# hugofloresgarcia/ddsp_pytorch

Hardware: NVIDIA B200
Metric: DDSP synth audio samples/sec (fwd+bwd) (higher is better)
Workload: dtype f32

## Files before the change

ddsp_pytorch_b200/csrc/noise.cu:

```cuda
#include "common.cuh"

namespace {

constexpr int kNoiseThreads = 128;

__device__ __forceinline__ void ir_design_row(const float *m, const float *ct, float *h, int NB,
                                              int tid, int nthr) {
    const int half = NB - 1, F = 2 * half;
    const float invF = 1.f / (float)F;
    for (int n = tid; 2 * n <= half; n += nthr) {
        float ev = 0.f, od = 0.f;
        int idx = 0;
        for (int k = 0; k < NB; ++k) {
            const float ck = (k == 0 || k == half) ? 1.f : 2.f;
            const float t = ck * m[k] * ct[idx];
            if (k & 1) od += t; else ev += t;
            idx += n;
            if (idx >= F) idx -= F;
        }
        h[n] = (ev + od) * invF;
        h[half - n] = (ev - od) * invF;
    }
}

__device__ __forceinline__ void ir_design_row_bwd(const float *dh, const float *ct, float *dm, int NB,
                                                  int tid, int nthr) {
    const int half = NB - 1, F = 2 * half;
    const float invF = 1.f / (float)F;
    for (int k = tid; k < NB; k += nthr) {
        float acc = 0.f;
        int idx = 0;
        for (int n = 0; n <= half; ++n) {
            acc = fmaf(dh[n], ct[idx], acc);
            idx += k;
            if (idx >= F) idx -= F;
        }
        dm[k] = acc * invF * ((k == 0 || k == half) ? 1.f : 2.f);
    }
}

__device__ __forceinline__ float hann_periodic(int i, int F) {
    return 0.5f - 0.5f * cospif(2.f * (float)i / (float)F);
}

template <bool BWD>
__global__ void __launch_bounds__(kNoiseThreads)
amp_to_ir_kernel(const float *__restrict__ in, float *__restrict__ out, int64_t rows, int NB,
                 int target) {
    extern __shared__ __align__(16) float smem[];
    const int half = NB - 1, F = 2 * half;
    float *ct = smem;
    float *m = ct + F;
    float *h = m + NB;
    const int tid = threadIdx.x;
    for (int i = tid; i < F; i += kNoiseThreads) ct[i] = cospif(2.f * (float)i / (float)F);
    const int lim = min(F, target);
    for (int64_t row = blockIdx.x; row < rows; row += gridDim.x) {
        __syncthreads();
        if (!BWD) {
            for (int k = tid; k < NB; k += kNoiseThreads) m[k] = in[row * NB + k];
            __syncthreads();
            ir_design_row(m, ct, h, NB, tid, kNoiseThreads);
            __syncthreads();
            for (int i = tid; i < target; i += kNoiseThreads) {
                int j = i + half;
                j = j % target;
                float v = 0.f;
                if (j < lim) {
                    int n = j - half;
                    if (n < 0) n += F;
                    n = min(n, F - n);
                    v = h[n] * hann_periodic(j, F);
                }
                out[row * target + i] = v;
            }
        } else {
            for (int n = tid; n <= half; n += kNoiseThreads) h[n] = 0.f;
            __syncthreads();
            for (int i = tid; i < target; i += kNoiseThreads) {
                int j = (i + half) % target;
                if (j < lim) {
                    int n = j - half;
                    if (n < 0) n += F;
                    n = min(n, F - n);
                    atomicAdd(&h[n], in[row * target + i] * hann_periodic(j, F));
                }
            }
            __syncthreads();
            ir_design_row_bwd(h, ct, m, NB, tid, kNoiseThreads);
            __syncthreads();
            for (int k = tid; k < NB; k += kNoiseThreads) out[row * NB + k] = m[k];
        }
    }
}

struct NoiseLayout {
    int NBp, HP, F, half, bs, stride;
    __host__ __device__ NoiseLayout(int NB, int bs_) {
        half = NB - 1; F = 2 * half; bs = bs_;
        NBp = (NB + 3) & ~3; HP = (half + 1 + 3) & ~3;
        stride = NBp + HP + F + (half + bs) + bs;
        stride = (stride + 3) & ~3;
    }
    __host__ __device__ int m() const { return 0; }
    __host__ __device__ int h() const { return NBp; }
    __host__ __device__ int taps() const { return NBp + HP; }
    __host__ __device__ int xs() const { return NBp + HP + F; }
    __host__ __device__ int ys() const { return NBp + HP + F + half + bs; }
};

__global__ void __launch_bounds__(kNoiseThreads)
filtered_noise_fwd_kernel(const float *__restrict__ mags, const float *__restrict__ noise,
                          const float *__restrict__ add, float *__restrict__ out, int64_t rows, int NB,
                          int bs, int RPC, int apply_scale, float bias) {
    extern __shared__ __align__(16) float smem[];
    const NoiseLayout L(NB, bs);
    const int half = L.half, F = L.F;
    float *ct = smem;
    float *rowbase = smem + ((F + 3) & ~3);
    const int tid = threadIdx.x;
    for (int i = tid; i < F; i += kNoiseThreads) ct[i] = cospif(2.f * (float)i / (float)F);

    const int QT = bs >> 2;
    for (int64_t r0 = (int64_t)blockIdx.x * RPC; r0 < rows; r0 += (int64_t)gridDim.x * RPC) {
        const int nr = (int)min((int64_t)RPC, rows - r0);
        __syncthreads();
        for (int i = tid; i < nr * NB; i += kNoiseThreads) {
            const int r = i / NB, k = i - r * NB;
            const float m = __ldg(mags + (r0 + r) * NB + k);
            rowbase[r * L.stride + L.m() + k] = apply_scale ? ddsp_scale_fn(m + bias) : m;
        }
        for (int i = tid; i < nr * (half + bs); i += kNoiseThreads) {
            const int r = i / (half + bs), j = i - r * (half + bs);
            rowbase[r * L.stride + L.xs() + j] = j < half ? 0.f : __ldg(noise + (r0 + r) * bs + (j - half));
        }
        __syncthreads();
        {
            const int per = kNoiseThreads / nr;
            const int r = tid / per, t = tid - r * per;
            if (r < nr) {
                float *rb = rowbase + r * L.stride;
                ir_design_row(rb + L.m(), ct, rb + L.h(), NB, t, per);
            }
        }
        __syncthreads();
        for (int i = tid; i < nr * F; i += kNoiseThreads) {
            const int r = i / F, d = i - r * F;
            float *rb = rowbase + r * L.stride;
            const float *h = rb + L.h();
            rb[L.taps() + d] = d < half ? h[d] * hann_periodic(d + half, F)
                                        : h[F - d] * hann_periodic(d - half, F);
        }
        __syncthreads();
        for (int w = tid; w < nr * QT; w += kNoiseThreads) {
            const int r = w / QT, i = (w - r * QT) * 4;
            const float *rb = rowbase + r * L.stride;
            const float4 *c4 = reinterpret_cast<const float4 *>(rb + L.taps());
            const float *xs = rb + L.xs() + half + i;
            float y0 = 0.f, y1 = 0.f, y2 = 0.f, y3 = 0.f;
            float4 hi = *reinterpret_cast<const float4 *>(xs);
            for (int d = 0; d < half; d += 4) {
                const float4 lo = *reinterpret_cast<const float4 *>(xs - d - 4);
                const float4 c = c4[d >> 2];
                y0 = fmaf(c.x, hi.x, y0); y1 = fmaf(c.x, hi.y, y1); y2 = fmaf(c.x, hi.z, y2); y3 = fmaf(c.x, hi.w, y3);
                y0 = fmaf(c.y, lo.w, y0); y1 = fmaf(c.y, hi.x, y1); y2 = fmaf(c.y, hi.y, y2); y3 = fmaf(c.y, hi.z, y3);
                y0 = fmaf(c.z, lo.z, y0); y1 = fmaf(c.z, lo.w, y1); y2 = fmaf(c.z, hi.x, y2); y3 = fmaf(c.z, hi.y, y3);
                y0 = fmaf(c.w, lo.y, y0); y1 = fmaf(c.w, lo.z, y1); y2 = fmaf(c.w, lo.w, y2); y3 = fmaf(c.w, hi.x, y3);
                hi = lo;
            }
            *reinterpret_cast<float4 *>(const_cast<float *>(rb) + L.ys() + i) = make_float4(y0, y1, y2, y3);
        }
        __syncthreads();
        for (int w = tid; w < nr * half; w += kNoiseThreads) {
            const int r = w / half, t = w - r * half;
            float *rb = rowbase + r * L.stride;
            const float *far = rb + L.taps() + half;
            const float *x = rb + L.xs() + half;
            float acc = 0.f;
            for (int e = 1; e <= t; ++e) acc = fmaf(far[e], x[t - e], acc);
            rb[L.ys() + bs - half + t] += acc;
        }
        __syncthreads();
        for (int i = tid; i < nr * bs; i += kNoiseThreads) {
            const int r = i / bs, j = i - r * bs;
            float y = rowbase[r * L.stride + L.ys() + j];
            if (add) y += __ldg(add + (r0 + r) * bs + j);
            out[(r0 + r) * bs + j] = y;
        }
    }
}

__global__ void __launch_bounds__(kNoiseThreads)
filtered_noise_bwd_kernel(const float *__restrict__ g_out, const float *__restrict__ noise,
                          const float *__restrict__ mags_raw, float *__restrict__ d_mags, int64_t rows,
                          int NB, int bs, int RPC, int apply_scale, float bias) {
    extern __shared__ __align__(16) float smem[];
    const NoiseLayout L(NB, bs);
    const int half = L.half, F = L.F;
    float *ct = smem;
    float *rowbase = smem + ((F + 3) & ~3);
    const int tid = threadIdx.x;
    for (int i = tid; i < F; i += kNoiseThreads) ct[i] = cospif(2.f * (float)i / (float)F);

    for (int64_t r0 = (int64_t)blockIdx.x * RPC; r0 < rows; r0 += (int64_t)gridDim.x * RPC) {
        const int nr = (int)min((int64_t)RPC, rows - r0);
        __syncthreads();
        for (int i = tid; i < nr * (half + bs); i += kNoiseThreads) {
            const int r = i / (half + bs), j = i - r * (half + bs);
            rowbase[r * L.stride + L.xs() + j] = j < half ? 0.f : __ldg(noise + (r0 + r) * bs + (j - half));
        }
        for (int i = tid; i < nr * bs; i += kNoiseThreads) {
            const int r = i / bs, j = i - r * bs;
            rowbase[r * L.stride + L.ys() + j] = __ldg(g_out + (r0 + r) * bs + j);
        }
        __syncthreads();
        for (int w = tid; w < nr * F; w += kNoiseThreads) {
            const int r = w / F, d = w - r * F;
            float *rb = rowbase + r * L.stride;
            const float *g = rb + L.ys();
            const float *x = rb + L.xs() + half;
            float a0 = 0.f, a1 = 0.f;
            if (d < half) {
                int i = 0;
                for (; i + 1 < bs; i += 2) {
                    a0 = fmaf(g[i], x[i - d], a0);
                    a1 = fmaf(g[i + 1], x[i + 1 - d], a1);
                }
                if (i < bs) a0 = fmaf(g[i], x[i - d], a0);
            } else {
                const int e = d - half;
                if (e >= 1)
                    for (int t = e; t < half; ++t) a0 = fmaf(g[bs - half + t], x[t - e], a0);
            }
            rb[L.taps() + d] = a0 + a1;
        }
        __syncthreads();
        for (int w = tid; w < nr * (half + 1); w += kNoiseThreads) {
            const int r = w / (half + 1), n = w - r * (half + 1);
            float *rb = rowbase + r * L.stride;
            const float *dt = rb + L.taps();
            float v = 0.f;
            if (n < half) v = dt[n] * hann_periodic(n + half, F);
            const int e = half - n;
            if (e >= 1 && e < half) v = fmaf(dt[half + e], hann_periodic(e, F), v);
            rb[L.h() + n] = v;
        }
        __syncthreads();
        {
            const int per = kNoiseThreads / nr;
            const int r = tid / per, t = tid - r * per;
            if (r < nr) {
                float *rb = rowbase + r * L.stride;
                ir_design_row_bwd(rb + L.h(), ct, rb + L.m(), NB, t, per);
            }
        }
        __syncthreads();
        for (int i = tid; i < nr * NB; i += kNoiseThreads) {
            const int r = i / NB, k = i - r * NB;
            float d = rowbase[r * L.stride + L.m() + k];
            if (apply_scale) d *= ddsp_scale_grad(__ldg(mags_raw + (r0 + r) * NB + k) + bias);
            d_mags[(r0 + r) * NB + k] = d;
        }
    }
}

constexpr int kN2Threads = 256;

__global__ void noise_design_kernel(float *__restrict__ tab, int NB) {
    const int half = NB - 1, F = 2 * half, NBq = (NB + 3) & ~3;
    const int total = NB * F;
    for (int i = blockIdx.x * blockDim.x + threadIdx.x; i < total; i += gridDim.x * blockDim.x) {
        const int k = i / F, j = i - k * F;
        const int n = j < half ? j : half - (j - half);
        const int wi = j < half ? j + half : j - half;
        const double ck = (k == 0 || k == half) ? 1.0 : 2.0;
        const double c = ck * cospi(2.0 * (double)((k * n) % F) / F) / F;
        const double w = 0.5 - 0.5 * cospi(2.0 * (double)wi / F);
        const float v = (float)(c * w);
        tab[i] = v;
        tab[(size_t)total + (size_t)j * NBq + k] = v;
    }
    for (int i = blockIdx.x * blockDim.x + threadIdx.x; i < F * (NBq - NB); i += gridDim.x * blockDim.x) {
        const int j = i / (NBq - NB), k = NB + i % (NBq - NB);
        tab[(size_t)total + (size_t)j * NBq + k] = 0.f;
    }
}

__device__ __forceinline__ float4 fir4(const float4 *__restrict__ t4, const float *x, int ntaps) {
    float y0 = 0.f, y1 = 0.f, y2 = 0.f, y3 = 0.f;
    float4 hi = *reinterpret_cast<const float4 *>(x);
    for (int d = 0; d < ntaps; d += 4) {
        const float4 lo = *reinterpret_cast<const float4 *>(x - d - 4);
        const float4 c = t4[d >> 2];
        y0 = fmaf(c.x, hi.x, y0); y1 = fmaf(c.x, hi.y, y1); y2 = fmaf(c.x, hi.z, y2); y3 = fmaf(c.x, hi.w, y3);
        y0 = fmaf(c.y, lo.w, y0); y1 = fmaf(c.y, hi.x, y1); y2 = fmaf(c.y, hi.y, y2); y3 = fmaf(c.y, hi.z, y3);
        y0 = fmaf(c.z, lo.z, y0); y1 = fmaf(c.z, lo.w, y1); y2 = fmaf(c.z, hi.x, y2); y3 = fmaf(c.z, hi.y, y3);
        y0 = fmaf(c.w, lo.y, y0); y1 = fmaf(c.w, lo.z, y1); y2 = fmaf(c.w, lo.w, y2); y3 = fmaf(c.w, hi.x, y3);
        hi = lo;
    }
    return make_float4(y0, y1, y2, y3);
}

__device__ __forceinline__ float4 corr4(const float *g, const float *x, int d, int len) {
    float a0 = 0.f, a1 = 0.f, a2 = 0.f, a3 = 0.f;
    float4 lo = *reinterpret_cast<const float4 *>(x - d - 4);
    for (int i = 0; i < len; i += 4) {
        const float4 hi = *reinterpret_cast<const float4 *>(x + i - d);
        const float4 gv = *reinterpret_cast<const float4 *>(g + i);
        a0 = fmaf(gv.x, hi.x, a0); a0 = fmaf(gv.y, hi.y, a0); a0 = fmaf(gv.z, hi.z, a0); a0 = fmaf(gv.w, hi.w, a0);
        a1 = fmaf(gv.x, lo.w, a1); a1 = fmaf(gv.y, hi.x, a1); a1 = fmaf(gv.z, hi.y, a1); a1 = fmaf(gv.w, hi.z, a1);
        a2 = fmaf(gv.x, lo.z, a2); a2 = fmaf(gv.y, lo.w, a2); a2 = fmaf(gv.z, hi.x, a2); a2 = fmaf(gv.w, hi.y, a2);
        a3 = fmaf(gv.x, lo.y, a3); a3 = fmaf(gv.y, lo.z, a3); a3 = fmaf(gv.z, lo.w, a3); a3 = fmaf(gv.w, hi.x, a3);
        lo = hi;
    }
    return make_float4(a0, a1, a2, a3);
}

struct Noise2Layout {
    int half, F, NBq, bs, xs_len, stride;
    __host__ __device__ Noise2Layout(int NB, int bs_) {
        half = NB - 1; F = 2 * half; NBq = (NB + 3) & ~3; bs = bs_;
        xs_len = half + bs;
        stride = NBq + F + xs_len + bs + half;
    }
    __host__ __device__ int m() const { return 0; }
    __host__ __device__ int taps() const { return NBq; }
    __host__ __device__ int xs() const { return NBq + F; }
    __host__ __device__ int ys() const { return NBq + F + xs_len; }
    __host__ __device__ int yf() const { return NBq + F + xs_len + bs; }
};

__global__ void __launch_bounds__(kN2Threads)
filtered_noise2_fwd_kernel(const float *__restrict__ mags, const float *__restrict__ noise,
                           const float *__restrict__ add, const float *__restrict__ design,
                           float *__restrict__ out, int64_t rows, int NB, int bs, int RPC, int apply_scale,
                           float bias) {
    extern __shared__ __align__(16) float smem[];
    const Noise2Layout L(NB, bs);
    const int half = L.half, F = L.F;
    float *D = smem;
    float *rowbase = D + NB * F;
    const int tid = threadIdx.x, warp = tid >> 5, lane = tid & 31;
    constexpr int NW = kN2Threads / 32;
    for (int i = tid; i < NB * F / 4; i += kN2Threads)
        reinterpret_cast<float4 *>(D)[i] = __ldg(reinterpret_cast<const float4 *>(design) + i);

    const int QM = bs >> 2, QF = half >> 2;
    for (int64_t r0 = (int64_t)blockIdx.x * RPC; r0 < rows; r0 += (int64_t)gridDim.x * RPC) {
        const int nr = (int)min((int64_t)RPC, rows - r0);
        __syncthreads();
        for (int r = warp; r < nr; r += NW) {
            float *rb = rowbase + r * L.stride;
            const float *mg = mags + (r0 + r) * NB;
            for (int k = lane; k < NB; k += 32) {
                const float m = __ldg(mg + k);
                rb[L.m() + k] = apply_scale ? ddsp_scale_fn(m + bias) : m;
            }
            for (int j = lane; j < half; j += 32) rb[L.xs() + j] = 0.f;
            const float4 *nz = reinterpret_cast<const float4 *>(noise + (r0 + r) * bs);
            float4 *xs4 = reinterpret_cast<float4 *>(rb + L.xs() + half);
            for (int j = lane; j < QM; j += 32) xs4[j] = __ldg(nz + j);
        }
        __syncthreads();
        for (int it = tid; it < ((nr + 1) >> 1) * (F / 4); it += kN2Threads) {
            const int rp = it / (F / 4), c = it - rp * (F / 4);
            const int ra = 2 * rp, rb_ = min(2 * rp + 1, nr - 1);
            const float *ma = rowbase + ra * L.stride + L.m();
            const float *mb = rowbase + rb_ * L.stride + L.m();
            const float4 *d4 = reinterpret_cast<const float4 *>(D) + c;
            float4 a = make_float4(0.f, 0.f, 0.f, 0.f), e = a;
#define DDSP_N2_MAC(X, Y, U)                                                                                  \
    a.x = fmaf(X, U.x, a.x); a.y = fmaf(X, U.y, a.y); a.z = fmaf(X, U.z, a.z); a.w = fmaf(X, U.w, a.w);      \
    e.x = fmaf(Y, U.x, e.x); e.y = fmaf(Y, U.y, e.y); e.z = fmaf(Y, U.z, e.z); e.w = fmaf(Y, U.w, e.w);
            for (int k = 0; k < NB - 1; k += 4) {
                const float4 xa = *reinterpret_cast<const float4 *>(ma + k);
                const float4 xb = *reinterpret_cast<const float4 *>(mb + k);
                const float4 u0 = d4[k * (F / 4)], u1 = d4[(k + 1) * (F / 4)];
                const float4 u2 = d4[(k + 2) * (F / 4)], u3 = d4[(k + 3) * (F / 4)];
                DDSP_N2_MAC(xa.x, xb.x, u0)
                DDSP_N2_MAC(xa.y, xb.y, u1)
                DDSP_N2_MAC(xa.z, xb.z, u2)
                DDSP_N2_MAC(xa.w, xb.w, u3)
            }
            {
                const float4 u = d4[(NB - 1) * (F / 4)];
                const float x = ma[NB - 1], y = mb[NB - 1];
                DDSP_N2_MAC(x, y, u)
            }
#undef DDSP_N2_MAC
            reinterpret_cast<float4 *>(rowbase + ra * L.stride + L.taps())[c] = a;
            if (rb_ != ra) reinterpret_cast<float4 *>(rowbase + rb_ * L.stride + L.taps())[c] = e;
        }
        __syncthreads();
        const int nmain = nr * QM;
        for (int it = tid; it < nmain + nr * QF; it += kN2Threads) {
            if (it < nmain) {
                const int r = it / QM, q = it - r * QM;
                float *rb = rowbase + r * L.stride;
                const float4 y = fir4(reinterpret_cast<const float4 *>(rb + L.taps()), rb + L.xs() + half + 4 * q, half);
                *reinterpret_cast<float4 *>(rb + L.ys() + 4 * q) = y;
            } else {
                const int i2 = it - nmain;
                const int r = i2 / QF, qq = i2 - r * QF;
                float *rb = rowbase + r * L.stride;
                const float4 y = fir4(reinterpret_cast<const float4 *>(rb + L.taps()) + QF,
                                      rb + L.xs() + half + 4 * qq, half);
                *reinterpret_cast<float4 *>(rb + L.yf() + 4 * qq) = y;
            }
        }
        __syncthreads();
        for (int r = warp; r < nr; r += NW) {
            const float *rb = rowbase + r * L.stride;
            const float4 *ys4 = reinterpret_cast<const float4 *>(rb + L.ys());
            const float4 *yf4 = reinterpret_cast<const float4 *>(rb + L.yf());
            const float4 *ad4 = add ? reinterpret_cast<const float4 *>(add + (r0 + r) * bs) : nullptr;
            float4 *o4 = reinterpret_cast<float4 *>(out + (r0 + r) * bs);
            for (int j = lane; j < QM; j += 32) {
                float4 y = ys4[j];
                if (j >= QM - QF) {
                    const float4 f = yf4[j - (QM - QF)];
                    y.x += f.x; y.y += f.y; y.z += f.z; y.w += f.w;
                }
                if (ad4) {
                    const float4 f = __ldg(ad4 + j);
                    y.x += f.x; y.y += f.y; y.z += f.z; y.w += f.w;
                }
                o4[j] = y;
            }
        }
    }
}

__global__ void __launch_bounds__(kN2Threads)
filtered_noise2_bwd_kernel(const float *__restrict__ g_out, const float *__restrict__ noise,
                           const float *__restrict__ mags_raw, const float *__restrict__ design,
                           float *__restrict__ d_mags, int64_t rows, int NB, int bs, int RPC,
                           int apply_scale, float bias) {
    extern __shared__ __align__(16) float smem[];
    const Noise2Layout L(NB, bs);
    const int half = L.half, F = L.F, NBq = L.NBq;
    float *Dt = smem;
    float *rowbase = Dt + F * NBq;
    const int tid = threadIdx.x, warp = tid >> 5, lane = tid & 31;
    constexpr int NW = kN2Threads / 32;
    const float *dt_src = design + (size_t)NB * F;
    for (int i = tid; i < F * NBq / 4; i += kN2Threads)
        reinterpret_cast<float4 *>(Dt)[i] = __ldg(reinterpret_cast<const float4 *>(dt_src) + i);
    const int QM = bs >> 2;

    for (int64_t r0 = (int64_t)blockIdx.x * RPC; r0 < rows; r0 += (int64_t)gridDim.x * RPC) {
        const int nr = (int)min((int64_t)RPC, rows - r0);
        __syncthreads();
        for (int r = warp; r < nr; r += NW) {
            float *rb = rowbase + r * L.stride;
            for (int j = lane; j < half; j += 32) rb[L.xs() + j] = 0.f;
            const float4 *nz = reinterpret_cast<const float4 *>(noise + (r0 + r) * bs);
            const float4 *gz = reinterpret_cast<const float4 *>(g_out + (r0 + r) * bs);
            float4 *xs4 = reinterpret_cast<float4 *>(rb + L.xs() + half);
            float4 *g4 = reinterpret_cast<float4 *>(rb + L.ys());
            for (int j = lane; j < QM; j += 32) {
                xs4[j] = __ldg(nz + j);
                g4[j] = __ldg(gz + j);
            }
        }
        __syncthreads();
        const int ncausal = nr * (half / 4);
        for (int it = tid; it < 2 * ncausal; it += kN2Threads) {
            const bool far = it >= ncausal;
            const int i2 = far ? it - ncausal : it;
            const int r = i2 / (half / 4), tg = i2 - r * (half / 4);
            float *rb = rowbase + r * L.stride;
            const float *x = rb + L.xs() + half;
            const float4 a = far ? corr4(rb + L.ys() + bs - half, x, 4 * tg, half) : corr4(rb + L.ys(), x, 4 * tg, bs);
            *reinterpret_cast<float4 *>(rb + L.taps() + (far ? half : 0) + 4 * tg) = a;
        }
        __syncthreads();
        for (int it = tid; it < ((nr + 1) >> 1) * (NBq / 4); it += kN2Threads) {
            const int rp = it / (NBq / 4), kg = it - rp * (NBq / 4);
            const int ra = 2 * rp, rb_ = min(2 * rp + 1, nr - 1);
            const float *ta = rowbase + ra * L.stride + L.taps();
            const float *tb = rowbase + rb_ * L.stride + L.taps();
            const float4 *d4 = reinterpret_cast<const float4 *>(Dt) + kg;
            float4 a = make_float4(0.f, 0.f, 0.f, 0.f), e = a;
#define DDSP_N2_MAC(X, Y, U)                                                                                  \
    a.x = fmaf(X, U.x, a.x); a.y = fmaf(X, U.y, a.y); a.z = fmaf(X, U.z, a.z); a.w = fmaf(X, U.w, a.w);      \
    e.x = fmaf(Y, U.x, e.x); e.y = fmaf(Y, U.y, e.y); e.z = fmaf(Y, U.z, e.z); e.w = fmaf(Y, U.w, e.w);
            for (int j = 0; j < F; j += 4) {
                const float4 xa = *reinterpret_cast<const float4 *>(ta + j);
                const float4 xb = *reinterpret_cast<const float4 *>(tb + j);
                const float4 u0 = d4[j * (NBq / 4)], u1 = d4[(j + 1) * (NBq / 4)];
                const float4 u2 = d4[(j + 2) * (NBq / 4)], u3 = d4[(j + 3) * (NBq / 4)];
                DDSP_N2_MAC(xa.x, xb.x, u0)
                DDSP_N2_MAC(xa.y, xb.y, u1)
                DDSP_N2_MAC(xa.z, xb.z, u2)
                DDSP_N2_MAC(xa.w, xb.w, u3)
            }
#undef DDSP_N2_MAC
#pragma unroll
            for (int h2 = 0; h2 < 2; ++h2) {
                if (h2 == 1 && rb_ == ra) break;
                const int r = h2 ? rb_ : ra;
                const float4 acc = h2 ? e : a;
                const float av[4] = {acc.x, acc.y, acc.z, acc.w};
#pragma unroll
                for (int q = 0; q < 4; ++q) {
                    const int k = 4 * kg + q;
                    if (k < NB) {
                        float d = av[q];
                        if (apply_scale) d *= ddsp_scale_grad(__ldg(mags_raw + (r0 + r) * NB + k) + bias);
                        d_mags[(r0 + r) * NB + k] = d;
                    }
                }
            }
        }
    }
}

inline int noise_rows_per_cta(int bs) {
    int rpc = (kNoiseThreads * 4) / bs;
    if (rpc < 1) rpc = 1;
    if (rpc > 8) rpc = 8;
    return rpc;
}

}

extern "C" int ddsp_b200_amp_to_ir_fwd(const float *amp, float *ir, int64_t rows, int NB, int target,
                                       void *stream) {
    DDSP_REQUIRE(amp && ir && rows >= 0 && NB >= 2 && target >= 1);
    if (rows == 0) return DDSP_B200_OK;
    const size_t smem = (size_t)(2 * (NB - 1) + NB + NB) * sizeof(float);
    if (smem > 48 * 1024) return DDSP_B200_EUNSUPPORTED;
    const int grid = (int)(rows < DDSP_SM_COUNT * 16 ? rows : DDSP_SM_COUNT * 16);
    amp_to_ir_kernel<false><<<grid, kNoiseThreads, smem, (cudaStream_t)stream>>>(amp, ir, rows, NB,
                                                                                 target);
    return ddsp_launch_status();
}

extern "C" int ddsp_b200_amp_to_ir_bwd(const float *d_ir, float *d_amp, int64_t rows, int NB,
                                       int target, void *stream) {
    DDSP_REQUIRE(d_ir && d_amp && rows >= 0 && NB >= 2 && target >= 1);
    if (rows == 0) return DDSP_B200_OK;
    const size_t smem = (size_t)(2 * (NB - 1) + NB + NB) * sizeof(float);
    if (smem > 48 * 1024) return DDSP_B200_EUNSUPPORTED;
    const int grid = (int)(rows < DDSP_SM_COUNT * 16 ? rows : DDSP_SM_COUNT * 16);
    amp_to_ir_kernel<true><<<grid, kNoiseThreads, smem, (cudaStream_t)stream>>>(d_ir, d_amp, rows,
                                                                                NB, target);
    return ddsp_launch_status();
}

static int noise_launch_cfg(int64_t rows, int NB, int bs, int *rpc, size_t *smem, int *grid) {
    if (NB < 3 || (NB - 1) % 4 != 0) return DDSP_B200_EUNSUPPORTED;
    if (bs % 4 != 0 || bs < 2 * (NB - 1)) return DDSP_B200_EUNSUPPORTED;
    *rpc = noise_rows_per_cta(bs);
    const NoiseLayout L(NB, bs);
    *smem = ((size_t)((L.F + 3) & ~3) + (size_t)*rpc * L.stride) * sizeof(float);
    if (*smem > 200 * 1024) return DDSP_B200_EUNSUPPORTED;
    const int64_t ctas = ddsp_ceil_div(rows, *rpc);
    *grid = (int)(ctas < DDSP_SM_COUNT * 8 ? ctas : DDSP_SM_COUNT * 8);
    return DDSP_B200_OK;
}

static bool noise2_cfg(int64_t rows, int NB, int bs, bool bwd, int *rpc, size_t *smem, int *grid) {
    if (NB < 5 || (NB - 1) % 4 != 0 || bs % 4 != 0 || bs < 2 * (NB - 1)) return false;
    const Noise2Layout L(NB, bs);
    const size_t fixed = (bwd ? (size_t)L.F * L.NBq : (size_t)NB * L.F) * sizeof(float);
    int r = 16;
    while (r > 1 && fixed + (size_t)r * L.stride * sizeof(float) > 75 * 1024) r >>= 1;
    *smem = fixed + (size_t)r * L.stride * sizeof(float);
    if (*smem > 200 * 1024) return false;
    *rpc = r;
    const int64_t ctas = ddsp_ceil_div(rows, r);
    *grid = (int)(ctas < DDSP_SM_COUNT * 3 ? ctas : DDSP_SM_COUNT * 3);
    return true;
}

extern "C" int64_t ddsp_b200_noise_design_size(int NB) {
    if (NB < 2) return 0;
    const int F = 2 * (NB - 1), NBq = (NB + 3) & ~3;
    return (int64_t)NB * F + (int64_t)F * NBq;
}

extern "C" int ddsp_b200_noise_design_table(float *table, int NB, void *stream) {
    DDSP_REQUIRE(table && NB >= 2);
    noise_design_kernel<<<64, 256, 0, (cudaStream_t)stream>>>(table, NB);
    return ddsp_launch_status();
}

extern "C" int ddsp_b200_filtered_noise_fwd(const float *mags, const float *noise, const float *add,
                                            const float *design, float *out, int64_t rows, int NB,
                                            int block_size, int apply_scale, float bias, void *stream) {
    DDSP_REQUIRE(mags && noise && out && rows >= 0);
    if (rows == 0) return DDSP_B200_OK;
    int rpc, grid;
    size_t smem;
    if (design && noise2_cfg(rows, NB, block_size, false, &rpc, &smem, &grid)) {
        if (smem > 48 * 1024)
            cudaFuncSetAttribute(filtered_noise2_fwd_kernel, cudaFuncAttributeMaxDynamicSharedMemorySize,
                                 (int)smem);
        filtered_noise2_fwd_kernel<<<grid, kN2Threads, smem, (cudaStream_t)stream>>>(
            mags, noise, add, design, out, rows, NB, block_size, rpc, apply_scale, bias);
        return ddsp_launch_status();
    }
    int s = noise_launch_cfg(rows, NB, block_size, &rpc, &smem, &grid);
    if (s) return s;
    if (smem > 48 * 1024)
        cudaFuncSetAttribute(filtered_noise_fwd_kernel, cudaFuncAttributeMaxDynamicSharedMemorySize,
                             (int)smem);
    filtered_noise_fwd_kernel<<<grid, kNoiseThreads, smem, (cudaStream_t)stream>>>(
        mags, noise, add, out, rows, NB, block_size, rpc, apply_scale, bias);
    return ddsp_launch_status();
}

extern "C" int ddsp_b200_filtered_noise_bwd(const float *g_out, const float *noise,
                                            const float *mags_raw, const float *design, float *d_mags,
                                            int64_t rows, int NB, int block_size, int apply_scale,
                                            float bias, void *stream) {
    DDSP_REQUIRE(g_out && noise && d_mags && rows >= 0 && (!apply_scale || mags_raw));
    if (rows == 0) return DDSP_B200_OK;
    int rpc, grid;
    size_t smem;
    if (design && noise2_cfg(rows, NB, block_size, true, &rpc, &smem, &grid)) {
        if (smem > 48 * 1024)
            cudaFuncSetAttribute(filtered_noise2_bwd_kernel, cudaFuncAttributeMaxDynamicSharedMemorySize,
                                 (int)smem);
        filtered_noise2_bwd_kernel<<<grid, kN2Threads, smem, (cudaStream_t)stream>>>(
            g_out, noise, mags_raw, design, d_mags, rows, NB, block_size, rpc, apply_scale, bias);
        return ddsp_launch_status();
    }
    int s = noise_launch_cfg(rows, NB, block_size, &rpc, &smem, &grid);
    if (s) return s;
    if (smem > 48 * 1024)
        cudaFuncSetAttribute(filtered_noise_bwd_kernel, cudaFuncAttributeMaxDynamicSharedMemorySize,
                             (int)smem);
    filtered_noise_bwd_kernel<<<grid, kNoiseThreads, smem, (cudaStream_t)stream>>>(
        g_out, noise, mags_raw, d_mags, rows, NB, block_size, rpc, apply_scale, bias);
    return ddsp_launch_status();
}
```

ddsp_pytorch_b200/csrc/torch_ops.cpp:

```cpp
#include <ATen/ATen.h>
#include <ATen/cuda/CUDAContext.h>
#include <ATen/cuda/CUDAEvent.h>
#include <c10/cuda/CUDAGuard.h>
#include <c10/cuda/CUDAStream.h>
#include <torch/library.h>

#include <map>
#include <mutex>
#include <tuple>
#include <vector>

#include "ddsp_b200.h"

namespace {

using at::Tensor;

void check(int status, const char *what) {
    TORCH_CHECK(status == DDSP_B200_OK, "ddsp_b200::", what, " failed: ", ddsp_b200_strerror(status),
                " (status ", status, ")");
}

Tensor prep(const Tensor &t, const char *name) {
    TORCH_CHECK(t.is_cuda(), "ddsp_b200: ", name, " must be a CUDA tensor (no CPU fallback exists)");
    TORCH_CHECK(t.scalar_type() == at::kFloat, "ddsp_b200: ", name, " must be float32, got ",
                t.scalar_type());
    return t.contiguous();
}

void *cur_stream() { return (void *)at::cuda::getCurrentCUDAStream().stream(); }
const float *fp(const Tensor &t) { return t.data_ptr<float>(); }
float *fpm(Tensor &t) { return t.data_ptr<float>(); }

void finish_table_build(const char *what) {
    cudaStreamCaptureStatus cap = cudaStreamCaptureStatusNone;
    cudaStream_t st = at::cuda::getCurrentCUDAStream().stream();
    TORCH_CHECK(cudaStreamIsCapturing(st, &cap) == cudaSuccess && cap == cudaStreamCaptureStatusNone,
                "ddsp_b200: constant table '", what, "' would be built inside a CUDA graph capture; run the op "
                "once eagerly (warm-up) before capturing");
    TORCH_CHECK(cudaStreamSynchronize(st) == cudaSuccess, "ddsp_b200: building table '", what, "' failed");
}

Tensor twiddle_table(const at::Device &dev, int64_t n) {
    static std::mutex mu;
    static std::map<std::pair<int, int64_t>, Tensor> cache;
    std::lock_guard<std::mutex> lock(mu);
    auto key = std::make_pair((int)dev.index(), n);
    auto it = cache.find(key);
    if (it != cache.end()) return it->second;
    Tensor t = at::empty({n, 2}, at::TensorOptions().device(dev).dtype(at::kFloat));
    check(ddsp_b200_twiddle_table(fpm(t), (int)n, cur_stream()), "twiddle_table");
    finish_table_build("twiddle_table");
    cache[key] = t;
    return t;
}

Tensor stage_twiddle_table(const at::Device &dev, int64_t n_fft) {
    static std::mutex mu;
    static std::map<std::pair<int, int64_t>, Tensor> cache;
    std::lock_guard<std::mutex> lock(mu);
    auto key = std::make_pair((int)dev.index(), n_fft);
    auto it = cache.find(key);
    if (it != cache.end()) return it->second;
    const int64_t n = ddsp_b200_fft_stage_twiddles_size((int)n_fft);
    Tensor t;
    if (n > 0) {
        t = at::empty({n, 2}, at::TensorOptions().device(dev).dtype(at::kFloat));
        check(ddsp_b200_fft_stage_twiddles(fpm(t), (int)n_fft, cur_stream()), "stft_stage_twiddles");
        finish_table_build("fft_stage_twiddles");
    }
    cache[key] = t;
    return t;
}

Tensor noise_design_table(const at::Device &dev, int64_t NB) {
    static std::mutex mu;
    static std::map<std::pair<int, int64_t>, Tensor> cache;
    std::lock_guard<std::mutex> lock(mu);
    auto key = std::make_pair((int)dev.index(), NB);
    auto it = cache.find(key);
    if (it != cache.end()) return it->second;
    Tensor t = at::empty({ddsp_b200_noise_design_size((int)NB)}, at::TensorOptions().device(dev).dtype(at::kFloat));
    check(ddsp_b200_noise_design_table(fpm(t), (int)NB, cur_stream()), "noise_design_table");
    finish_table_build("noise_design_table");
    cache[key] = t;
    return t;
}

Tensor scale_function_fwd(const Tensor &x_) {
    Tensor x = prep(x_, "x");
    c10::cuda::CUDAGuard guard(x.device());
    Tensor y = at::empty_like(x);
    check(ddsp_b200_scale_function_fwd(fp(x), fpm(y), x.numel(), cur_stream()), "scale_function_fwd");
    return y;
}

Tensor scale_function_bwd(const Tensor &x_, const Tensor &dy_) {
    Tensor x = prep(x_, "x"), dy = prep(dy_, "dy");
    TORCH_CHECK(x.numel() == dy.numel(), "scale_function_bwd: size mismatch");
    c10::cuda::CUDAGuard guard(x.device());
    Tensor dx = at::empty_like(x);
    check(ddsp_b200_scale_function_bwd(fp(x), fp(dy), fpm(dx), x.numel(), cur_stream()),
          "scale_function_bwd");
    return dx;
}

Tensor remove_above_nyquist(const Tensor &amp_, const Tensor &f0_, double sample_rate) {
    Tensor amp = prep(amp_, "amplitudes"), f0 = prep(f0_, "f0");
    TORCH_CHECK(amp.dim() >= 1 && f0.numel() * amp.size(-1) == amp.numel(),
                "remove_above_nyquist: f0 must have one value per row of amplitudes");
    c10::cuda::CUDAGuard guard(amp.device());
    Tensor out = at::empty_like(amp);
    check(ddsp_b200_remove_above_nyquist(fp(amp), fp(f0), fpm(out), f0.numel(), (int)amp.size(-1),
                                         (float)sample_rate, cur_stream()),
          "remove_above_nyquist");
    return out;
}

Tensor opt_prep(const c10::optional<Tensor> &t, const char *name) {
    return (t.has_value() && t->defined()) ? prep(*t, name) : Tensor();
}
const float *opt_fp(const Tensor &t) { return t.defined() ? t.data_ptr<float>() : nullptr; }

std::tuple<Tensor, Tensor, Tensor> harmonic_controls_fwd(const Tensor &amp_raw_, const Tensor &dist_raw_,
                                                         const Tensor &f0_, double sample_rate,
                                                         bool with_weights) {
    Tensor a = prep(amp_raw_, "amplitudes"), d = prep(dist_raw_, "harmonic_distribution"),
           f = prep(f0_, "f0");
    const int64_t H = d.size(-1), rows = d.numel() / H;
    TORCH_CHECK(a.numel() == rows && f.numel() == rows, "harmonic_controls: shape mismatch");
    c10::cuda::CUDAGuard guard(d.device());
    Tensor amps = at::empty_like(a), dist = at::empty_like(d);
    Tensor weights = with_weights ? at::empty_like(d) : at::empty({0}, d.options());
    check(ddsp_b200_harmonic_controls_fwd(fp(a), fp(d), fp(f), fpm(amps), fpm(dist),
                                          with_weights ? fpm(weights) : nullptr, rows, (int)H,
                                          (float)sample_rate, cur_stream()),
          "harmonic_controls_fwd");
    return {amps, dist, weights};
}

std::tuple<Tensor, Tensor> harmonic_controls_bwd(const Tensor &amp_raw_, const Tensor &dist_raw_,
                                                 const Tensor &f0_, const c10::optional<Tensor> &d_amps_,
                                                 const c10::optional<Tensor> &d_dist_,
                                                 const c10::optional<Tensor> &d_weights_,
                                                 double sample_rate) {
    Tensor a = prep(amp_raw_, "amplitudes"), d = prep(dist_raw_, "harmonic_distribution"),
           f = prep(f0_, "f0");
    Tensor ga = opt_prep(d_amps_, "d_amps"), gd = opt_prep(d_dist_, "d_dist"),
           gw = opt_prep(d_weights_, "d_weights");
    const int64_t H = d.size(-1), rows = d.numel() / H;
    TORCH_CHECK(a.numel() == rows && f.numel() == rows && (!ga.defined() || ga.numel() == rows) &&
                    (!gd.defined() || gd.numel() == d.numel()) && (!gw.defined() || gw.numel() == d.numel()),
                "harmonic_controls_bwd: shape mismatch");
    c10::cuda::CUDAGuard guard(d.device());
    Tensor da = at::empty_like(a), dd = at::empty_like(d);
    check(ddsp_b200_harmonic_controls_bwd(fp(a), fp(d), fp(f), opt_fp(ga), opt_fp(gd), opt_fp(gw), fpm(da),
                                          fpm(dd), rows, (int)H, (float)sample_rate, cur_stream()),
          "harmonic_controls_bwd");
    return {da, dd};
}

std::tuple<Tensor, Tensor, Tensor, Tensor> harmonic_fwd(const Tensor &f0_, const Tensor &weights_,
                                                        int64_t block_size, double sample_rate,
                                                        const c10::optional<Tensor> &phase0_) {
    Tensor f0 = prep(f0_, "f0"), w = prep(weights_, "weights");
    TORCH_CHECK(w.dim() == 3, "harmonic_fwd: weights must be (B,T,H)");
    const int64_t B = w.size(0), T = w.size(1), H = w.size(2);
    TORCH_CHECK(f0.numel() == B * T, "harmonic_fwd: f0 must be (B,T,1)");
    c10::cuda::CUDAGuard guard(w.device());
    auto opt64 = w.options().dtype(at::kLong);
    Tensor phi = at::empty({B, T}, opt64), delta = at::empty({B, T}, opt64);
    Tensor phase_end = at::empty({B}, w.options().dtype(at::kDouble));
    Tensor audio = at::empty({B, T * block_size, 1}, w.options());
    if (B == 0 || T == 0) return {audio, phase_end.zero_(), phi, delta};
    const double *p0 = nullptr;
    Tensor phase0;
    if (phase0_.has_value() && phase0_->defined()) {
        phase0 = phase0_->contiguous();
        TORCH_CHECK(phase0.is_cuda() && phase0.scalar_type() == at::kDouble && phase0.numel() == B,
                    "harmonic_fwd: phase0 must be a CUDA float64 tensor of B turns");
        p0 = phase0.data_ptr<double>();
    }
    check(ddsp_b200_phase_scan(fp(f0), p0, (uint64_t *)phi.data_ptr<int64_t>(),
                               (uint64_t *)delta.data_ptr<int64_t>(), phase_end.data_ptr<double>(),
                               (int)B, (int)T, (int)block_size, sample_rate, cur_stream()),
          "phase_scan");
    check(ddsp_b200_harmonic_frames_fwd(fp(w), (const uint64_t *)phi.data_ptr<int64_t>(),
                                        (const uint64_t *)delta.data_ptr<int64_t>(), fpm(audio), (int)B,
                                        (int)T, (int)H, (int)block_size, cur_stream()),
          "harmonic_frames_fwd");
    return {audio, phase_end, phi, delta};
}

std::tuple<Tensor, Tensor> harmonic_bwd(const Tensor &g_, const Tensor &weights_, const Tensor &phi,
                                        const Tensor &delta, int64_t block_size, double sample_rate,
                                        bool need_f0) {
    Tensor g = prep(g_, "grad_audio"), w = prep(weights_, "weights");
    const int64_t B = w.size(0), T = w.size(1), H = w.size(2);
    TORCH_CHECK(g.numel() == B * T * block_size, "harmonic_bwd: grad shape mismatch");
    TORCH_CHECK(phi.is_cuda() && phi.scalar_type() == at::kLong && phi.is_contiguous() &&
                    delta.is_cuda() && delta.scalar_type() == at::kLong && delta.is_contiguous() &&
                    phi.numel() == B * T && delta.numel() == B * T,
                "harmonic_bwd: bad phase workspace");
    c10::cuda::CUDAGuard guard(w.device());
    Tensor dw = at::empty_like(w);
    if (B == 0 || T == 0) return {dw, at::empty({B, T, 1}, w.options())};
    const uint64_t *ph = (const uint64_t *)phi.data_ptr<int64_t>();
    const uint64_t *dl = (const uint64_t *)delta.data_ptr<int64_t>();
    check(ddsp_b200_harmonic_frames_bwd_weights(fp(g), ph, dl, fpm(dw), (int)B, (int)T, (int)H,
                                                (int)block_size, cur_stream()),
          "harmonic_frames_bwd_weights");
    Tensor df0;
    if (need_f0) {
        df0 = at::empty({B, T, 1}, w.options());
        Tensor scratch = at::empty({B, T, 2}, w.options());
        check(ddsp_b200_harmonic_frames_bwd_f0(fp(g), fp(w), ph, dl, fpm(scratch), fpm(df0), (int)B, (int)T,
                                               (int)H, (int)block_size, sample_rate, cur_stream()),
              "harmonic_frames_bwd_f0");
    } else {
        df0 = at::empty({0}, w.options());
    }
    return {dw, df0};
}

int64_t harmonic_raw_supported(int64_t H, int64_t block_size) {
    return ddsp_b200_harmonic_frames_raw_supported((int)H, (int)block_size);
}

struct RawViews {
    Tensor first, dist;
    const float *amp, *dst;
    int64_t amp_stride, dist_stride, B, T, H;
    bool joint;
};

RawViews raw_views(const Tensor &first_, const c10::optional<Tensor> &dist_raw_) {
    RawViews v;
    v.first = prep(first_, "amplitudes / projection");
    v.joint = !(dist_raw_.has_value() && dist_raw_->defined());
    TORCH_CHECK(v.first.dim() == 3, "harmonic_raw: expected (B,T,.) tensors");
    v.B = v.first.size(0);
    v.T = v.first.size(1);
    if (v.joint) {
        v.H = v.first.size(2) - 1;
        TORCH_CHECK(v.H >= 1, "harmonic_raw: the projection must be (B,T,H+1)");
        v.amp = fp(v.first);
        v.dst = v.amp + 1;
        v.amp_stride = v.dist_stride = v.H + 1;
    } else {
        v.dist = prep(*dist_raw_, "harmonic_distribution");
        TORCH_CHECK(v.dist.dim() == 3 && v.dist.size(0) == v.B && v.dist.size(1) == v.T && v.first.size(2) == 1,
                    "harmonic_raw: amplitudes (B,T,1) and harmonic_distribution (B,T,H) expected");
        v.H = v.dist.size(2);
        v.amp = fp(v.first);
        v.dst = fp(v.dist);
        v.amp_stride = 1;
        v.dist_stride = v.H;
    }
    return v;
}

std::tuple<Tensor, Tensor, Tensor, Tensor, Tensor, Tensor> harmonic_raw_fwd(
    const Tensor &first_, const c10::optional<Tensor> &dist_raw_, const Tensor &f0_, int64_t block_size,
    double sample_rate, const c10::optional<Tensor> &phase0_) {
    RawViews v = raw_views(first_, dist_raw_);
    Tensor f0 = prep(f0_, "f0");
    const int64_t B = v.B, T = v.T, H = v.H;
    TORCH_CHECK(f0.numel() == B * T, "harmonic_raw_fwd: f0 must be (B,T,1)");
    c10::cuda::CUDAGuard guard(f0.device());
    auto opt = f0.options();
    Tensor phi = at::empty({B, T}, opt.dtype(at::kLong)), delta = at::empty({B, T}, opt.dtype(at::kLong));
    Tensor phase_end = at::empty({B}, opt.dtype(at::kDouble));
    Tensor audio = at::empty({B, T * block_size, 1}, opt);
    Tensor amps = at::empty({B, T, 1}, opt), weights = at::empty({B, T, H}, opt);
    if (B == 0 || T == 0) return {audio, phase_end.zero_(), phi, delta, amps, weights};
    const double *p0 = nullptr;
    Tensor phase0;
    if (phase0_.has_value() && phase0_->defined()) {
        phase0 = phase0_->contiguous();
        TORCH_CHECK(phase0.is_cuda() && phase0.scalar_type() == at::kDouble && phase0.numel() == B,
                    "harmonic_raw_fwd: phase0 must be a CUDA float64 tensor of B turns");
        p0 = phase0.data_ptr<double>();
    }
    check(ddsp_b200_harmonic_frames_raw_scan_fwd(v.amp, v.amp_stride, v.dst, v.dist_stride, fp(f0), p0,
                                                 (uint64_t *)phi.data_ptr<int64_t>(),
                                                 (uint64_t *)delta.data_ptr<int64_t>(), phase_end.data_ptr<double>(),
                                                 fpm(amps), fpm(weights), fpm(audio), (int)B, (int)T, (int)H,
                                                 (int)block_size, sample_rate, cur_stream()),
          "harmonic_frames_raw_scan_fwd");
    return {audio, phase_end, phi, delta, amps, weights};
}

std::tuple<Tensor, Tensor> harmonic_raw_bwd(const Tensor &g_, const Tensor &first_,
                                            const c10::optional<Tensor> &dist_raw_, const Tensor &f0_,
                                            const Tensor &phi, const Tensor &delta, int64_t block_size,
                                            double sample_rate) {
    RawViews v = raw_views(first_, dist_raw_);
    Tensor g = prep(g_, "grad_audio"), f0 = prep(f0_, "f0");
    const int64_t B = v.B, T = v.T, H = v.H;
    TORCH_CHECK(g.numel() == B * T * block_size && f0.numel() == B * T, "harmonic_raw_bwd: shape mismatch");
    TORCH_CHECK(phi.is_cuda() && phi.scalar_type() == at::kLong && phi.is_contiguous() &&
                    delta.is_cuda() && delta.scalar_type() == at::kLong && delta.is_contiguous() &&
                    phi.numel() == B * T && delta.numel() == B * T,
                "harmonic_raw_bwd: bad phase workspace");
    c10::cuda::CUDAGuard guard(g.device());
    Tensor d0, d1;
    float *da, *dd;
    int64_t das, dds;
    if (v.joint) {
        d0 = at::empty({B, T, H + 1}, g.options());
        d1 = at::empty({0}, g.options());
        da = fpm(d0);
        dd = da + 1;
        das = dds = H + 1;
    } else {
        d0 = at::empty({B, T, 1}, g.options());
        d1 = at::empty({B, T, H}, g.options());
        da = fpm(d0);
        dd = fpm(d1);
        das = 1;
        dds = H;
    }
    if (B == 0 || T == 0) return {d0, d1};
    check(ddsp_b200_harmonic_frames_raw_bwd(fp(g), v.amp, v.amp_stride, v.dst, v.dist_stride, fp(f0),
                                            (const uint64_t *)phi.data_ptr<int64_t>(),
                                            (const uint64_t *)delta.data_ptr<int64_t>(), da, das, dd, dds, (int)B,
                                            (int)T, (int)H, (int)block_size, (float)sample_rate, cur_stream()),
          "harmonic_frames_raw_bwd");
    return {d0, d1};
}

std::tuple<Tensor, Tensor> harmonic_ar_fwd(const Tensor &f0_, const Tensor &amps_, double sample_rate) {
    Tensor f0 = prep(f0_, "f0"), a = prep(amps_, "amplitudes");
    TORCH_CHECK(a.dim() == 3, "harmonic_synth: amplitudes must be (B,N,H)");
    const int64_t B = a.size(0), N = a.size(1), H = a.size(2);
    TORCH_CHECK(f0.numel() == B * N, "harmonic_synth: f0 must be (B,N,1)");
    c10::cuda::CUDAGuard guard(a.device());
    Tensor phase = at::empty({B, N}, a.options().dtype(at::kLong));
    Tensor audio = at::empty({B, N, 1}, a.options());
    check(ddsp_b200_phase_scan_audio_rate(fp(f0), (uint64_t *)phase.data_ptr<int64_t>(), (int)B, N,
                                          sample_rate, cur_stream()),
          "phase_scan_audio_rate");
    check(ddsp_b200_harmonic_audio_rate_fwd(fp(a), (const uint64_t *)phase.data_ptr<int64_t>(), fpm(audio),
                                            (int)B, N, (int)H, cur_stream()),
          "harmonic_audio_rate_fwd");
    return {audio, phase};
}

std::tuple<Tensor, Tensor> harmonic_ar_bwd(const Tensor &g_, const Tensor &amps_, const Tensor &phase,
                                           double sample_rate, bool need_f0) {
    Tensor g = prep(g_, "grad_audio"), a = prep(amps_, "amplitudes");
    const int64_t B = a.size(0), N = a.size(1), H = a.size(2);
    TORCH_CHECK(g.numel() == B * N && phase.numel() == B * N && phase.scalar_type() == at::kLong &&
                    phase.is_cuda() && phase.is_contiguous(),
                "harmonic_synth backward: shape mismatch");
    c10::cuda::CUDAGuard guard(a.device());
    Tensor da = at::empty_like(a);
    Tensor df0 = need_f0 ? at::empty({B, N, 1}, a.options()) : at::empty({0}, a.options());
    Tensor dphi = need_f0 ? at::empty({B, N}, a.options()) : Tensor();
    check(ddsp_b200_harmonic_audio_rate_bwd(fp(g), fp(a), (const uint64_t *)phase.data_ptr<int64_t>(),
                                            fpm(da), need_f0 ? fpm(dphi) : nullptr,
                                            need_f0 ? fpm(df0) : nullptr, (int)B, N, (int)H, sample_rate,
                                            cur_stream()),
          "harmonic_audio_rate_bwd");
    return {da, df0};
}

Tensor amp_to_ir_fwd(const Tensor &amp_, int64_t target) {
    Tensor amp = prep(amp_, "amp");
    const int64_t NB = amp.size(-1), rows = amp.numel() / NB;
    c10::cuda::CUDAGuard guard(amp.device());
    auto shape = amp.sizes().vec();
    shape.back() = target;
    Tensor ir = at::empty(shape, amp.options());
    check(ddsp_b200_amp_to_ir_fwd(fp(amp), fpm(ir), rows, (int)NB, (int)target, cur_stream()),
          "amp_to_ir_fwd");
    return ir;
}

Tensor amp_to_ir_bwd(const Tensor &d_ir_, int64_t NB) {
    Tensor d_ir = prep(d_ir_, "d_ir");
    const int64_t target = d_ir.size(-1), rows = d_ir.numel() / target;
    c10::cuda::CUDAGuard guard(d_ir.device());
    auto shape = d_ir.sizes().vec();
    shape.back() = NB;
    Tensor d_amp = at::empty(shape, d_ir.options());
    check(ddsp_b200_amp_to_ir_bwd(fp(d_ir), fpm(d_amp), rows, (int)NB, (int)target, cur_stream()),
          "amp_to_ir_bwd");
    return d_amp;
}

Tensor noise_fwd(const Tensor &mags_, const Tensor &noise_, const c10::optional<Tensor> &add_, bool apply_scale,
                 double bias) {
    Tensor mags = prep(mags_, "magnitudes"), noise = prep(noise_, "noise"), add = opt_prep(add_, "add");
    TORCH_CHECK(mags.dim() == 3 && noise.dim() == 3 && mags.size(0) == noise.size(0) &&
                    mags.size(1) == noise.size(1),
                "filtered noise: magnitudes (B,T,NB) and noise (B,T,block) expected");
    const int64_t B = mags.size(0), T = mags.size(1), NB = mags.size(2), bs = noise.size(2);
    TORCH_CHECK(!add.defined() || add.numel() == B * T * bs, "filtered noise: `add` must be (B,T*block,1)");
    c10::cuda::CUDAGuard guard(mags.device());
    Tensor out = at::empty({B, T * bs, 1}, mags.options());
    if (B * T == 0) return out;
    Tensor design = noise_design_table(mags.device(), NB);
    check(ddsp_b200_filtered_noise_fwd(fp(mags), fp(noise), opt_fp(add), fp(design), fpm(out), B * T, (int)NB,
                                       (int)bs, apply_scale, (float)bias, cur_stream()),
          "filtered_noise_fwd");
    return out;
}

Tensor noise_bwd(const Tensor &g_, const Tensor &noise_, const c10::optional<Tensor> &mags_raw_, int64_t NB,
                 bool apply_scale, double bias) {
    Tensor g = prep(g_, "grad_out"), noise = prep(noise_, "noise"), raw = opt_prep(mags_raw_, "mags_raw");
    const int64_t B = noise.size(0), T = noise.size(1), bs = noise.size(2);
    TORCH_CHECK(g.numel() == B * T * bs, "filtered noise backward: shape mismatch");
    TORCH_CHECK(!apply_scale || (raw.defined() && raw.numel() == B * T * NB),
                "filtered noise backward: raw magnitudes needed when the scale function is fused");
    c10::cuda::CUDAGuard guard(noise.device());
    Tensor d_mags = at::empty({B, T, NB}, noise.options());
    if (B * T == 0) return d_mags;
    Tensor design = noise_design_table(noise.device(), NB);
    check(ddsp_b200_filtered_noise_bwd(fp(g), fp(noise), opt_fp(raw), fp(design), fpm(d_mags), B * T, (int)NB,
                                       (int)bs, apply_scale, (float)bias, cur_stream()),
          "filtered_noise_bwd");
    return d_mags;
}

struct ConvPlan {
    int n1, n2;
    int64_t n;
    Tensor tw, st1, st2;
};

ConvPlan conv_plan(const at::Device &dev, int64_t min_len) {
    ConvPlan p;
    check(ddsp_b200_conv_plan(min_len, &p.n1, &p.n2), "conv_plan");
    p.n = (int64_t)p.n1 * p.n2;
    p.tw = twiddle_table(dev, p.n);
    p.st1 = stage_twiddle_table(dev, p.n1);
    p.st2 = stage_twiddle_table(dev, p.n2);
    return p;
}

Tensor fftconv_spectrum(const Tensor &kernel_, int64_t n_signal) {
    Tensor ker = prep(kernel_, "kernel");
    TORCH_CHECK(ker.dim() == 2 && n_signal > 0, "fftconv_spectrum: 2-D (rows, length) kernel expected");
    const int64_t Rk = ker.size(0), Lk = ker.size(1);
    c10::cuda::CUDAGuard guard(ker.device());
    const int64_t Lc = std::min(Lk, n_signal);
    Tensor kc = Lc == Lk ? ker : ker.narrow(1, 0, Lc).contiguous();
    ConvPlan p = conv_plan(ker.device(), n_signal + Lc - 1);
    void *st = cur_stream();
    Tensor hspec = at::empty({Rk, p.n, 2}, ker.options());
    check(ddsp_b200_fft4_cols_fwd(fp(kc), Rk, Lc, 0, fpm(hspec), fp(p.tw), opt_fp(p.st1), p.n1, p.n2, st), "fft4_cols_fwd(h)");
    check(ddsp_b200_fft4_rows_spectrum(fpm(hspec), Rk, fp(p.tw), fp(p.st2), p.n1, p.n2, st), "fft4_rows_spectrum");
    return hspec;
}

std::tuple<Tensor, Tensor, Tensor> fftconv_fwd(const Tensor &signal_, const Tensor &kernel_, bool keep,
                                               const c10::optional<Tensor> &hspec_,
                                               const c10::optional<Tensor> &signal2_) {
    Tensor sig = prep(signal_, "signal"), ker = prep(kernel_, "kernel");
    Tensor sig2 = opt_prep(signal2_, "signal2");
    TORCH_CHECK(!sig2.defined() || sig2.sizes() == sig.sizes(), "fftconv: signal2 must have the signal's shape");
    TORCH_CHECK(sig.dim() == 2 && ker.dim() == 2, "fftconv: 2-D (rows, length) tensors expected");
    const int64_t R = sig.size(0), n = sig.size(1), Rk = ker.size(0), Lk = ker.size(1);
    TORCH_CHECK(Rk == 1 || Rk == R, "fftconv: kernel rows must be 1 or match the signal rows");
    c10::cuda::CUDAGuard guard(sig.device());
    Tensor out = at::empty_like(sig);
    Tensor none = at::empty({0}, sig.options());
    if (R == 0 || n == 0) return {out, none, none};
    const int64_t Lc = std::min(Lk, n);
    ConvPlan p = conv_plan(sig.device(), n + Lc - 1);
    const int pair = Rk == 1;
    const int64_t slots = pair ? (R + 1) / 2 : R;
    void *st = cur_stream();
    Tensor hspec;
    if (hspec_.has_value() && hspec_->defined()) {
        hspec = prep(*hspec_, "hspec");
        TORCH_CHECK(hspec.numel() == Rk * p.n * 2, "fftconv: hspec does not belong to this kernel / signal length");
    } else {
        hspec = fftconv_spectrum(ker, n);
    }
    Tensor work = at::empty({slots, p.n, 2}, sig.options());
    check(ddsp_b200_fft4_cols_fwd_sum(fp(sig), opt_fp(sig2), R, n, pair, fpm(work), fp(p.tw), opt_fp(p.st1), p.n1, p.n2, st),
          "fft4_cols_fwd(x)");
    Tensor filtered = keep ? at::empty_like(work) : work;
    check(ddsp_b200_fft4_rows_filter(fp(work), fpm(filtered), slots, fp(hspec), pair ? 0 : p.n, 0, fp(p.tw), fp(p.st2),
                                     p.n1, p.n2, st),
          "fft4_rows_filter");
    check(ddsp_b200_fft4_cols_inv(fp(filtered), fpm(out), R, n, pair, opt_fp(p.st1), p.n1, p.n2, st), "fft4_cols_inv");
    if (keep) return {out, work, hspec};
    return {out, none, none};
}

std::tuple<Tensor, Tensor, Tensor> fftconv_bwd_parts(const Tensor &g_, const Tensor &signal_, const Tensor &kernel_,
                                                     const c10::optional<Tensor> &work_x_,
                                                     const c10::optional<Tensor> &hspec_,
                                                     const c10::optional<Tensor> &work_g_, bool need_signal,
                                                     bool need_kernel) {
    Tensor g = prep(g_, "grad_out"), sig = prep(signal_, "signal"), ker = prep(kernel_, "kernel");
    const int64_t R = sig.size(0), n = sig.size(1), Rk = ker.size(0), Lk = ker.size(1);
    TORCH_CHECK(g.dim() == 2 && g.size(0) == R && g.size(1) == n, "fftconv backward: grad shape mismatch");
    c10::cuda::CUDAGuard guard(sig.device());
    Tensor d_sig = need_signal ? at::empty_like(sig) : at::empty({0}, sig.options());
    Tensor d_ker = need_kernel ? at::zeros_like(ker) : at::empty({0}, sig.options());
    if (R == 0 || n == 0 || (!need_signal && !need_kernel)) return {d_sig, d_ker, at::empty({0}, sig.options())};
    const int64_t Lc = std::min(Lk, n);
    Tensor kc = Lc == Lk ? ker : ker.narrow(1, 0, Lc).contiguous();
    ConvPlan p = conv_plan(sig.device(), n + Lc - 1);
    const int pair = Rk == 1;
    const int64_t slots = pair ? (R + 1) / 2 : R;
    auto main_stream = at::cuda::getCurrentCUDAStream();
    void *st = (void *)main_stream.stream();
    const bool fork = need_kernel && need_signal;
    at::cuda::CUDAStream side = fork ? at::cuda::getStreamFromPool(false, sig.device().index()) : main_stream;
    void *ss = (void *)side.stream();
    Tensor scratch;
    int counters_zeroed = 0;
    if (need_kernel) {
        scratch = at::empty({ddsp_b200_fft4_correlate_splits_plan(slots, pair, p.n1, p.n2), p.n, 2}, sig.options());
        const int64_t coff = ddsp_b200_fft4_correlate_counter_offset(slots, pair, p.n1, p.n2);
        if (fork && coff >= 0) {
            at::cuda::CUDAEvent begun;
            begun.record(main_stream);
            begun.block(side);
            c10::cuda::CUDAStreamGuard sg(side);
            scratch.view({-1}).narrow(0, coff, p.n1).zero_();
            counters_zeroed = 1;
        }
    }
    Tensor work_g;
    if (work_g_.has_value() && work_g_->defined() && work_g_->numel() == slots * p.n * 2) {
        work_g = *work_g_;
        TORCH_CHECK(work_g.is_cuda() && work_g.scalar_type() == at::kFloat && work_g.is_contiguous(),
                    "fftconv backward: bad work_g");
    } else {
        work_g = at::empty({slots, p.n, 2}, sig.options());
        check(ddsp_b200_fft4_cols_fwd(fp(g), R, n, pair, fpm(work_g), fp(p.tw), opt_fp(p.st1), p.n1, p.n2, st), "fft4_cols_fwd(g)");
    }
    Tensor hspec = (hspec_.has_value() && hspec_->defined() && hspec_->numel() == Rk * p.n * 2) ? *hspec_ : Tensor();
    Tensor saved_x = (work_x_.has_value() && work_x_->defined() && work_x_->numel() == slots * p.n * 2) ? *work_x_ : Tensor();
    if (need_signal && !hspec.defined()) {
        hspec = at::empty({Rk, p.n, 2}, sig.options());
        check(ddsp_b200_fft4_cols_fwd(fp(kc), Rk, Lc, 0, fpm(hspec), fp(p.tw), opt_fp(p.st1), p.n1, p.n2, st), "fft4_cols_fwd(h)");
        check(ddsp_b200_fft4_rows_spectrum(fpm(hspec), Rk, fp(p.tw), fp(p.st2), p.n1, p.n2, st), "fft4_rows_spectrum");
    }
    at::cuda::CUDAEvent corr_done;
    if (need_kernel) {
        if (fork) {
            at::cuda::CUDAEvent g_ready;
            g_ready.record(main_stream);
            g_ready.block(side);
        }
        Tensor work_x = saved_x;
        if (!work_x.defined()) {
            work_x = at::empty({slots, p.n, 2}, sig.options());
            check(ddsp_b200_fft4_cols_fwd(fp(sig), R, n, pair, fpm(work_x), fp(p.tw), opt_fp(p.st1), p.n1, p.n2, ss),
                  "fft4_cols_fwd(x)");
        }
        Tensor corr = at::empty({Rk, p.n, 2}, sig.options());
        check(ddsp_b200_fft4_rows_correlate_ex(fp(work_g), fp(work_x), slots, pair, fpm(scratch), fpm(corr),
                                               fp(p.tw), fp(p.st2), p.n1, p.n2, counters_zeroed, ss),
              "fft4_rows_correlate");
        if (fork) corr_done.record(side);
        Tensor dk = Lc == Lk ? d_ker : at::empty({Rk, Lc}, sig.options());
        check(ddsp_b200_fft4_cols_inv(fp(corr), fpm(dk), Rk, Lc, 0, opt_fp(p.st1), p.n1, p.n2, ss), "fft4_cols_inv(dh)");
        if (Lc != Lk) {
            c10::cuda::CUDAStreamGuard sg(side);
            d_ker.narrow(1, 0, Lc).copy_(dk);
        }
    }
    if (need_signal) {
        if (fork) corr_done.block(main_stream);
        check(ddsp_b200_fft4_rows_filter(fp(work_g), fpm(work_g), slots, fp(hspec), pair ? 0 : p.n, 1, fp(p.tw), fp(p.st2),
                                         p.n1, p.n2, st),
              "fft4_rows_filter(conj)");
        check(ddsp_b200_fft4_cols_inv(fp(work_g), fpm(d_sig), R, n, pair, opt_fp(p.st1), p.n1, p.n2, st),
              "fft4_cols_inv(dx)");
    }
    if (fork) {
        at::cuda::CUDAEvent join;
        join.record(side);
        join.block(main_stream);
    }
    return {d_sig, d_ker, work_g};
}

std::tuple<Tensor, Tensor> fftconv_bwd(const Tensor &g, const Tensor &signal, const Tensor &kernel,
                                       const c10::optional<Tensor> &work_x, const c10::optional<Tensor> &hspec,
                                       bool need_signal, bool need_kernel) {
    auto r = fftconv_bwd_parts(g, signal, kernel, work_x, hspec, c10::nullopt, need_signal, need_kernel);
    return {std::get<0>(r), std::get<1>(r)};
}

Tensor reverb_impulse_fwd(const Tensor &noise_, const Tensor &decay_, const Tensor &wet_, const Tensor &t_) {
    Tensor noise = prep(noise_, "noise"), decay = prep(decay_, "decay"), wet = prep(wet_, "wet"),
           t = prep(t_, "t");
    const int64_t L = noise.numel();
    TORCH_CHECK(t.numel() == L && decay.numel() == 1 && wet.numel() == 1, "reverb impulse: shape mismatch");
    c10::cuda::CUDAGuard guard(noise.device());
    Tensor imp = at::empty({1, L, 1}, noise.options());
    check(ddsp_b200_reverb_impulse_fwd(fp(noise), fp(decay), fp(wet), fp(t), fpm(imp), (int)L, cur_stream()),
          "reverb_impulse_fwd");
    return imp;
}

std::tuple<Tensor, Tensor, Tensor> reverb_impulse_bwd(const Tensor &d_imp_, const Tensor &noise_,
                                                      const Tensor &decay_, const Tensor &wet_,
                                                      const Tensor &t_) {
    Tensor d_imp = prep(d_imp_, "d_impulse"), noise = prep(noise_, "noise"), decay = prep(decay_, "decay"),
           wet = prep(wet_, "wet"), t = prep(t_, "t");
    const int64_t L = noise.numel();
    TORCH_CHECK(d_imp.numel() <= L, "reverb impulse backward: d_impulse longer than the impulse");
    c10::cuda::CUDAGuard guard(noise.device());
    Tensor dn = at::empty_like(noise), dd = at::empty_like(decay), dw = at::empty_like(wet);
    Tensor scratch = at::empty({ddsp_b200_reverb_impulse_bwd_scratch() / 8}, noise.options().dtype(at::kDouble));
    check(ddsp_b200_reverb_impulse_bwd(fp(d_imp), (int)d_imp.numel(), fp(noise), fp(decay), fp(wet), fp(t),
                                       fpm(dn), fpm(dd), fpm(dw), (int)L, scratch.data_ptr(), cur_stream()),
          "reverb_impulse_bwd");
    return {dn, dd, dw};
}

int64_t pow2_ge(int64_t v) {
    int64_t p = 1;
    while (p < v) p <<= 1;
    return p;
}

Tensor stft_mag_fwd(const Tensor &signal_, const Tensor &window_, int64_t n_fft, int64_t hop) {
    Tensor sig = prep(signal_, "signal"), win = prep(window_, "window");
    TORCH_CHECK(sig.dim() == 2 && win.numel() == n_fft, "stft_mag: signal (B,N) and window (n_fft) expected");
    const int64_t B = sig.size(0), N = sig.size(1);
    c10::cuda::CUDAGuard guard(sig.device());
    Tensor tw = twiddle_table(sig.device(), std::max<int64_t>(4096, n_fft));
    Tensor mag = at::empty({B, n_fft / 2 + 1, 1 + N / hop}, sig.options());
    Tensor stw = stage_twiddle_table(sig.device(), n_fft);
    check(ddsp_b200_stft_mag_fwd(fp(sig), fp(win), fp(tw), (int)tw.size(0), stw.defined() ? fp(stw) : nullptr, fpm(mag),
                                 (int)B, N, (int)n_fft, (int)hop, cur_stream()),
          "stft_mag_fwd");
    return mag;
}

Tensor stft_mag_bwd(const Tensor &signal_, const Tensor &d_mag_, const Tensor &window_, int64_t n_fft,
                    int64_t hop) {
    Tensor sig = prep(signal_, "signal"), gm = prep(d_mag_, "d_mag"), win = prep(window_, "window");
    const int64_t B = sig.size(0), N = sig.size(1);
    TORCH_CHECK(gm.numel() == B * (n_fft / 2 + 1) * (1 + N / hop), "stft_mag backward: shape mismatch");
    c10::cuda::CUDAGuard guard(sig.device());
    Tensor tw = twiddle_table(sig.device(), std::max<int64_t>(4096, n_fft));
    Tensor d_sig = at::empty_like(sig);
    Tensor edge = at::empty({B, n_fft}, sig.options());
    void *st = cur_stream();
    Tensor stw = stage_twiddle_table(sig.device(), n_fft);
    check(ddsp_b200_stft_mag_bwd(fp(sig), fp(gm), fp(win), fp(tw), (int)tw.size(0), stw.defined() ? fp(stw) : nullptr,
                                 fpm(d_sig), fpm(edge), (int)B, N, (int)n_fft, (int)hop, 0, st),
          "stft_mag_bwd");
    const int sc = (int)n_fft;
    check(ddsp_b200_stft_fold_edges(fp(edge), fpm(d_sig), (int)B, N, &sc, 1, st), "stft_fold_edges");
    return d_sig;
}

std::tuple<Tensor, Tensor> mss_loss_fwd(const Tensor &target_, const Tensor &rec_, at::IntArrayRef scales,
                                        double overlap, const Tensor &windows_, bool need_grad) {
    Tensor tgt = prep(target_, "target"), rec = prep(rec_, "rec"), win = prep(windows_, "windows");
    TORCH_CHECK(tgt.dim() == 2 && rec.sizes() == tgt.sizes(), "mss_loss: target and rec must both be (B,N)");
    const int64_t B = rec.size(0), N = rec.size(1);
    const int ns = (int)scales.size();
    TORCH_CHECK(ns >= 1 && ns <= 8, "mss_loss: 1..8 scales supported");
    std::vector<int> sc(ns), hp(ns);
    int64_t wsum = 0, tiles = 0, esum = 0, smax = 0;
    for (int i = 0; i < ns; ++i) {
        sc[i] = (int)scales[i];
        hp[i] = (int)((double)scales[i] * (1.0 - overlap));
        const int64_t t = ddsp_b200_mss_tiles((int)B, N, sc[i], hp[i]);
        TORCH_CHECK(t > 0, "mss_loss: scale ", sc[i], " with hop ", hp[i], " unsupported for N=", N);
        tiles += t * B;
        wsum += sc[i];
        esum += B * sc[i];
        smax = std::max<int64_t>(smax, sc[i]);
    }
    TORCH_CHECK(win.numel() == wsum, "mss_loss: windows must hold sum(scales) values");
    c10::cuda::CUDAGuard guard(rec.device());
    if (ddsp_b200_mss_fused_supported(sc.data(), hp.data(), ns)) {
        int64_t ws_floats = 0, part_floats = 0;
        check(ddsp_b200_mss_fused_sizes((int)B, N, sc.data(), ns, &ws_floats, &part_floats), "mss_fused_sizes");
        std::vector<Tensor> tables;
        std::vector<const float *> tabs;
        for (int i = 0; i < ns; ++i) {
            tables.push_back(stage_twiddle_table(rec.device(), sc[i]));
            tabs.push_back(fp(tables.back()));
        }
        Tensor partial = at::empty({part_floats}, rec.options());
        Tensor loss = at::empty({}, rec.options());
        Tensor d_rec = need_grad ? at::empty_like(rec) : at::empty({0}, rec.options());
        Tensor ws = need_grad ? at::empty({ws_floats}, rec.options()) : Tensor();
        check(ddsp_b200_mss_fused(fp(tgt), fp(rec), fp(win), tabs.data(), need_grad ? fpm(ws) : nullptr, fpm(partial),
                                  need_grad ? fpm(d_rec) : nullptr, fpm(loss), (int)B, N, sc.data(), ns, cur_stream()),
              "mss_fused");
        return {loss, d_rec};
    }
    Tensor tw = twiddle_table(rec.device(), std::max<int64_t>(4096, pow2_ge(smax)));
    Tensor partial = at::empty({tiles, 2}, rec.options());
    Tensor loss = at::empty({}, rec.options());
    Tensor d_rec = need_grad ? at::empty_like(rec) : at::empty({0}, rec.options());
    Tensor edge = need_grad ? at::empty({esum}, rec.options()) : Tensor();
    Tensor d_scales = need_grad ? at::empty({ns, B, N}, rec.options()) : Tensor();
    auto main_stream = at::cuda::getCurrentCUDAStream();
    std::vector<Tensor> stage_tables;
    for (int i = 0; i < ns; ++i) stage_tables.push_back(stage_twiddle_table(rec.device(), sc[i]));
    std::vector<at::cuda::CUDAStream> streams;
    streams.push_back(main_stream);
    for (int i = 1; i < ns; ++i) streams.push_back(at::cuda::getStreamFromPool(false, rec.device().index()));
    at::cuda::CUDAEvent fork;
    fork.record(main_stream);
    for (int i = 1; i < ns; ++i) fork.block(streams[i]);
    int64_t woff = 0, poff = 0, eoff = 0;
    for (int i = 0; i < ns; ++i) {
        const Tensor &stw = stage_tables[i];
        check(ddsp_b200_mss_scale(fp(tgt), fp(rec), fp(win) + woff, fp(tw), (int)tw.size(0),
                                  stw.defined() ? fp(stw) : nullptr, fpm(partial) + 2 * poff,
                                  need_grad ? fpm(d_scales) + (int64_t)i * B * N : nullptr,
                                  need_grad ? fpm(edge) + eoff : nullptr, (int)B, N, sc[i], hp[i], 0,
                                  (void *)streams[i].stream()),
              "mss_scale");
        woff += sc[i];
        poff += ddsp_b200_mss_tiles((int)B, N, sc[i], hp[i]) * B;
        eoff += B * sc[i];
    }
    for (int i = 1; i < ns; ++i) {
        at::cuda::CUDAEvent join;
        join.record(streams[i]);
        join.block(main_stream);
    }
    check(ddsp_b200_mss_finish(fp(partial), need_grad ? fp(edge) : nullptr, need_grad ? fp(d_scales) : nullptr,
                               need_grad ? fpm(d_rec) : nullptr, fpm(loss), (int)B, N, sc.data(), hp.data(), ns,
                               (void *)main_stream.stream()),
          "mss_finish");
    return {loss, d_rec};
}

int64_t gru_supported(int64_t hidden) {
    if (hidden != 512) return 0;
    const int clusters = ddsp_b200_gru_resident_clusters();
    return clusters > 0 ? (int64_t)clusters * 10 : 0;
}

std::tuple<Tensor, Tensor> gru_fwd(const Tensor &gi_, const Tensor &w_hh_, const Tensor &b_hh_,
                                   const c10::optional<Tensor> &h0_, bool save_gates) {
    Tensor gi = prep(gi_, "gi"), w = prep(w_hh_, "weight_hh"), b = prep(b_hh_, "bias_hh"), h0 = opt_prep(h0_, "h0");
    TORCH_CHECK(gi.dim() == 3 && gi.size(2) % 3 == 0, "gru_fwd: gi must be (B,T,3H)");
    const int64_t B = gi.size(0), T = gi.size(1), H = gi.size(2) / 3;
    TORCH_CHECK(w.numel() == 3 * H * H && b.numel() == 3 * H && (!h0.defined() || h0.numel() == B * H),
                "gru_fwd: weight / bias / h0 shape mismatch");
    c10::cuda::CUDAGuard guard(gi.device());
    Tensor y = at::empty({B, T, H}, gi.options());
    Tensor gates = save_gates ? at::empty({B, T, 4 * H}, gi.options()) : at::empty({0}, gi.options());
    if (B == 0 || T == 0) return {y, gates};
    check(ddsp_b200_gru_fwd(fp(gi), fp(w), fp(b), opt_fp(h0), fpm(y), save_gates ? fpm(gates) : nullptr, (int)B,
                            (int)T, (int)H, cur_stream()),
          "gru_fwd");
    return {y, gates};
}

std::tuple<Tensor, Tensor, Tensor> gru_bwd(const Tensor &dy_, const c10::optional<Tensor> &dhT_, const Tensor &w_hh_,
                                           const Tensor &y_, const c10::optional<Tensor> &h0_, const Tensor &gates_) {
    Tensor dy = prep(dy_, "dy"), w = prep(w_hh_, "weight_hh"), y = prep(y_, "y"), gates = prep(gates_, "gates");
    Tensor dhT = opt_prep(dhT_, "dhT"), h0 = opt_prep(h0_, "h0");
    const int64_t B = y.size(0), T = y.size(1), H = y.size(2);
    TORCH_CHECK(dy.numel() == y.numel() && gates.numel() == 4 * y.numel(), "gru_bwd: shape mismatch");
    c10::cuda::CUDAGuard guard(y.device());
    Tensor dgi = at::empty({B, T, 3 * H}, y.options()), dgh = at::empty({B, T, 3 * H}, y.options());
    Tensor dh0 = at::empty({B, H}, y.options());
    if (B == 0 || T == 0) return {dgi, dgh, dh0.zero_()};
    check(ddsp_b200_gru_bwd(fp(dy), opt_fp(dhT), fp(w), fp(y), opt_fp(h0), fp(gates), fpm(dgi), fpm(dgh), fpm(dh0),
                            (int)B, (int)T, (int)H, cur_stream()),
          "gru_bwd");
    return {dgi, dgh, dh0};
}

Tensor gemm3x_split(const Tensor &x_, bool transpose) {
    Tensor x = prep(x_, "x");
    TORCH_CHECK(x.dim() == 2, "gemm3x_split: x must be 2-D");
    const int64_t rows = x.size(0), cols = x.size(1);
    const int64_t R = transpose ? cols : rows, K = transpose ? rows : cols;
    const int64_t Rp = transpose ? R : (R + 63) / 64 * 64;
    c10::cuda::CUDAGuard guard(x.device());
    Tensor out = at::empty({3 * Rp, ddsp_b200_gemm3x_ld(K)}, x.options().dtype(at::kBFloat16));
    if (rows == 0 || cols == 0) return out.zero_();
    check(ddsp_b200_gemm3x_split(fp(x), rows, cols, cols, transpose ? 1 : 0, out.data_ptr(), Rp, cur_stream()), "gemm3x_split");
    return out;
}

std::tuple<Tensor, Tensor> gemm3x_split_colsum(const Tensor &x_) {
    Tensor x = prep(x_, "x");
    TORCH_CHECK(x.dim() == 2, "gemm3x_split_colsum: x must be 2-D");
    const int64_t rows = x.size(0), cols = x.size(1), Rp = (rows + 63) / 64 * 64;
    c10::cuda::CUDAGuard guard(x.device());
    Tensor out = at::empty({3 * Rp, ddsp_b200_gemm3x_ld(cols)}, x.options().dtype(at::kBFloat16));
    Tensor colsum = at::empty({cols}, x.options());
    if (rows == 0 || cols == 0) return {out.zero_(), colsum.zero_()};
    Tensor partial = at::empty({ddsp_b200_gemm3x_colsum_scratch(Rp, cols)}, x.options());
    check(ddsp_b200_gemm3x_split_colsum(fp(x), rows, cols, cols, out.data_ptr(), Rp, fpm(colsum), fpm(partial), cur_stream()),
          "gemm3x_split_colsum");
    return {out, colsum};
}

std::tuple<Tensor, Tensor> gemm3x_split_both(const Tensor &x_) {
    Tensor x = prep(x_, "x");
    TORCH_CHECK(x.dim() == 2, "gemm3x_split_both: x must be 2-D");
    const int64_t rows = x.size(0), cols = x.size(1);
    c10::cuda::CUDAGuard guard(x.device());
    Tensor out = at::empty({3 * rows, ddsp_b200_gemm3x_ld(cols)}, x.options().dtype(at::kBFloat16));
    Tensor out_t = at::empty({3 * cols, ddsp_b200_gemm3x_ld(rows)}, x.options().dtype(at::kBFloat16));
    if (rows == 0 || cols == 0) return {out.zero_(), out_t.zero_()};
    check(ddsp_b200_gemm3x_split_both(fp(x), rows, cols, cols, out.data_ptr(), rows, out_t.data_ptr(), cols, cur_stream()),
          "gemm3x_split_both");
    return {out, out_t};
}

Tensor gemm3x_mm(const Tensor &a, const Tensor &b, int64_t M, int64_t N, int64_t K, const c10::optional<Tensor> &bias_,
                 bool a_mn, bool b_mn) {
    Tensor bias = opt_prep(bias_, "bias");
    TORCH_CHECK(a.is_cuda() && b.is_cuda() && a.scalar_type() == at::kBFloat16 && b.scalar_type() == at::kBFloat16 &&
                    a.is_contiguous() && b.is_contiguous() && a.dim() == 2 && b.dim() == 2 && a.size(0) % 3 == 0 &&
                    b.size(0) % 3 == 0,
                "gemm3x_mm: operands must be gemm3x_split outputs");
    const int64_t a_pr = a.size(0) / 3, b_pr = b.size(0) / 3;
    TORCH_CHECK(a_mn ? (a_pr >= K && a_pr % 64 == 0 && a.size(1) >= M) : (a_pr >= M && a.size(1) >= K),
                "gemm3x_mm: operand a does not hold an ", M, " x ", K, " matrix in the stated orientation");
    TORCH_CHECK(b_mn ? (b_pr >= K && b_pr % 64 == 0 && b.size(1) >= N) : (b_pr >= N && b.size(1) >= K),
                "gemm3x_mm: operand b does not hold an ", N, " x ", K, " matrix in the stated orientation");
    TORCH_CHECK(!bias.defined() || bias.numel() == N, "gemm3x_mm: bias must have N entries");
    c10::cuda::CUDAGuard guard(a.device());
    auto fopt = a.options().dtype(at::kFloat);
    Tensor c = at::empty({M, N}, fopt);
    if (M == 0 || N == 0) return c;
    if (K == 0) return bias.defined() ? c.copy_(bias.expand({M, N})) : c.zero_();
    const int splits = ddsp_b200_gemm3x_splits((int)M, (int)N, (int)K);
    Tensor ws = splits > 1 ? at::empty({splits, M, N}, fopt) : Tensor();
    check(ddsp_b200_gemm3x(a.data_ptr(), a_pr, a.size(1), a_mn ? 1 : 0, b.data_ptr(), b_pr, b.size(1), b_mn ? 1 : 0,
                           opt_fp(bias), fpm(c), N, (int)M, (int)N, (int)K, splits > 1 ? fpm(ws) : nullptr, cur_stream()),
          "gemm3x_mm");
    return c;
}

int64_t ln_lrelu_supported(int64_t n) { return n % 128 == 0 && n >= 128 && n <= 512; }

std::tuple<Tensor, Tensor> ln_lrelu_fwd(const Tensor &x_, const Tensor &gamma_, const Tensor &beta_, double eps,
                                        double slope, bool save_stats) {
    Tensor x = prep(x_, "x"), gamma = prep(gamma_, "weight"), beta = prep(beta_, "bias");
    const int64_t N = x.size(-1), rows = N ? x.numel() / N : 0;
    TORCH_CHECK(gamma.numel() == N && beta.numel() == N, "ln_lrelu_fwd: weight / bias must have N entries");
    c10::cuda::CUDAGuard guard(x.device());
    Tensor y = at::empty_like(x);
    Tensor stats = save_stats ? at::empty({rows, 2}, x.options()) : at::empty({0}, x.options());
    check(ddsp_b200_ln_lrelu_fwd(fp(x), fp(gamma), fp(beta), fpm(y), save_stats ? fpm(stats) : nullptr, rows, (int)N,
                                 (float)eps, (float)slope, cur_stream()),
          "ln_lrelu_fwd");
    return {y, stats};
}

std::tuple<Tensor, Tensor, Tensor> ln_lrelu_bwd(const Tensor &dy_, const Tensor &x_, const Tensor &gamma_,
                                                const Tensor &beta_, const Tensor &stats_, double slope) {
    Tensor dy = prep(dy_, "dy"), x = prep(x_, "x"), gamma = prep(gamma_, "weight"), beta = prep(beta_, "bias");
    Tensor stats = prep(stats_, "stats");
    const int64_t N = x.size(-1), rows = N ? x.numel() / N : 0;
    TORCH_CHECK(dy.numel() == x.numel() && stats.numel() == 2 * rows, "ln_lrelu_bwd: shape mismatch");
    c10::cuda::CUDAGuard guard(x.device());
    Tensor dx = at::empty_like(x), dg = at::empty({N}, x.options()), db = at::empty({N}, x.options());
    if (rows == 0) return {dx, dg.zero_(), db.zero_()};
    Tensor partial = at::empty({ddsp_b200_ln_lrelu_slots(rows), 2 * N}, x.options());
    check(ddsp_b200_ln_lrelu_bwd(fp(dy), fp(x), fp(gamma), fp(beta), fp(stats), fpm(dx), fpm(dg), fpm(db), fpm(partial),
                                 rows, (int)N, (float)slope, cur_stream()),
          "ln_lrelu_bwd");
    return {dx, dg, db};
}

int64_t abi_version() { return ddsp_b200_abi_version(); }

}

TORCH_LIBRARY(ddsp_b200, m) {
    m.def("abi_version() -> int", abi_version);
    m.def("gru_supported(int hidden) -> int", gru_supported);
    m.def("ln_lrelu_supported(int n) -> int", ln_lrelu_supported);
    m.def("ln_lrelu_fwd(Tensor x, Tensor weight, Tensor bias, float eps, float slope, bool save_stats) -> (Tensor, Tensor)");
    m.def("ln_lrelu_bwd(Tensor dy, Tensor x, Tensor weight, Tensor bias, Tensor stats, float slope) -> (Tensor, Tensor, Tensor)");
    m.def("gemm3x_split(Tensor x, bool transpose) -> Tensor");
    m.def("gemm3x_split_both(Tensor x) -> (Tensor, Tensor)");
    m.def("gemm3x_split_colsum(Tensor x) -> (Tensor, Tensor)");
    m.def("gemm3x_mm(Tensor a, Tensor b, int M, int N, int K, Tensor? bias, bool a_mn, bool b_mn) -> Tensor");
    m.def("gru_fwd(Tensor gi, Tensor weight_hh, Tensor bias_hh, Tensor? h0, bool save_gates) -> (Tensor, Tensor)");
    m.def("gru_bwd(Tensor dy, Tensor? dhT, Tensor weight_hh, Tensor y, Tensor? h0, Tensor gates) -> (Tensor, Tensor, Tensor)");
    m.def("scale_function_fwd(Tensor x) -> Tensor");
    m.def("scale_function_bwd(Tensor x, Tensor dy) -> Tensor");
    m.def("remove_above_nyquist(Tensor amplitudes, Tensor f0, float sample_rate) -> Tensor");
    m.def("harmonic_controls_fwd(Tensor amplitudes, Tensor harmonic_distribution, Tensor f0, float sample_rate, bool with_weights) -> (Tensor, Tensor, Tensor)");
    m.def("harmonic_controls_bwd(Tensor amplitudes, Tensor harmonic_distribution, Tensor f0, Tensor? d_amps, Tensor? d_dist, Tensor? d_weights, float sample_rate) -> (Tensor, Tensor)");
    m.def("harmonic_fwd(Tensor f0, Tensor weights, int block_size, float sample_rate, Tensor? phase0) -> (Tensor, Tensor, Tensor, Tensor)");
    m.def("harmonic_bwd(Tensor grad_audio, Tensor weights, Tensor phi, Tensor delta, int block_size, float sample_rate, bool need_f0) -> (Tensor, Tensor)");
    m.def("harmonic_raw_supported(int n_harmonic, int block_size) -> int", harmonic_raw_supported);
    m.def("harmonic_raw_fwd(Tensor first, Tensor? dist_raw, Tensor f0, int block_size, float sample_rate, Tensor? phase0) -> (Tensor, Tensor, Tensor, Tensor, Tensor, Tensor)");
    m.def("harmonic_raw_bwd(Tensor grad_audio, Tensor first, Tensor? dist_raw, Tensor f0, Tensor phi, Tensor delta, int block_size, float sample_rate) -> (Tensor, Tensor)");
    m.def("harmonic_ar_fwd(Tensor f0, Tensor amplitudes, float sample_rate) -> (Tensor, Tensor)");
    m.def("harmonic_ar_bwd(Tensor grad_audio, Tensor amplitudes, Tensor phase, float sample_rate, bool need_f0) -> (Tensor, Tensor)");
    m.def("amp_to_ir_fwd(Tensor amp, int target_size) -> Tensor");
    m.def("amp_to_ir_bwd(Tensor d_ir, int n_bands) -> Tensor");
    m.def("noise_fwd(Tensor magnitudes, Tensor noise, Tensor? add, bool apply_scale, float bias) -> Tensor");
    m.def("noise_bwd(Tensor grad_out, Tensor noise, Tensor? magnitudes_raw, int n_bands, bool apply_scale, float bias) -> Tensor");
    m.def("fftconv_spectrum(Tensor kernel, int n_signal) -> Tensor");
    m.def("fftconv_fwd(Tensor signal, Tensor kernel, bool keep_transforms, Tensor? hspec=None, Tensor? signal2=None) -> (Tensor, Tensor, Tensor)");
    m.def("fftconv_bwd(Tensor grad_out, Tensor signal, Tensor kernel, Tensor? work_x, Tensor? hspec, bool need_signal, bool need_kernel) -> (Tensor, Tensor)");
    m.def("fftconv_bwd_parts(Tensor grad_out, Tensor signal, Tensor kernel, Tensor? work_x, Tensor? hspec, Tensor? work_g, bool need_signal, bool need_kernel) -> (Tensor, Tensor, Tensor)");
    m.def("reverb_impulse_fwd(Tensor noise, Tensor decay, Tensor wet, Tensor t) -> Tensor");
    m.def("reverb_impulse_bwd(Tensor d_impulse, Tensor noise, Tensor decay, Tensor wet, Tensor t) -> (Tensor, Tensor, Tensor)");
    m.def("stft_mag_fwd(Tensor signal, Tensor window, int n_fft, int hop) -> Tensor");
    m.def("stft_mag_bwd(Tensor signal, Tensor d_mag, Tensor window, int n_fft, int hop) -> Tensor");
    m.def("mss_loss_fwd(Tensor target, Tensor rec, int[] scales, float overlap, Tensor windows, bool need_grad) -> (Tensor, Tensor)");
}

TORCH_LIBRARY_IMPL(ddsp_b200, CUDA, m) {
    m.impl("ln_lrelu_fwd", ln_lrelu_fwd);
    m.impl("ln_lrelu_bwd", ln_lrelu_bwd);
    m.impl("gemm3x_split", gemm3x_split);
    m.impl("gemm3x_split_both", gemm3x_split_both);
    m.impl("gemm3x_split_colsum", gemm3x_split_colsum);
    m.impl("gemm3x_mm", gemm3x_mm);
    m.impl("gru_fwd", gru_fwd);
    m.impl("gru_bwd", gru_bwd);
    m.impl("scale_function_fwd", scale_function_fwd);
    m.impl("scale_function_bwd", scale_function_bwd);
    m.impl("remove_above_nyquist", remove_above_nyquist);
    m.impl("harmonic_controls_fwd", harmonic_controls_fwd);
    m.impl("harmonic_controls_bwd", harmonic_controls_bwd);
    m.impl("harmonic_fwd", harmonic_fwd);
    m.impl("harmonic_bwd", harmonic_bwd);
    m.impl("harmonic_raw_fwd", harmonic_raw_fwd);
    m.impl("harmonic_raw_bwd", harmonic_raw_bwd);
    m.impl("harmonic_ar_fwd", harmonic_ar_fwd);
    m.impl("harmonic_ar_bwd", harmonic_ar_bwd);
    m.impl("amp_to_ir_fwd", amp_to_ir_fwd);
    m.impl("amp_to_ir_bwd", amp_to_ir_bwd);
    m.impl("noise_fwd", noise_fwd);
    m.impl("noise_bwd", noise_bwd);
    m.impl("fftconv_spectrum", fftconv_spectrum);
    m.impl("fftconv_fwd", fftconv_fwd);
    m.impl("fftconv_bwd", fftconv_bwd);
    m.impl("fftconv_bwd_parts", fftconv_bwd_parts);
    m.impl("reverb_impulse_fwd", reverb_impulse_fwd);
    m.impl("reverb_impulse_bwd", reverb_impulse_bwd);
    m.impl("stft_mag_fwd", stft_mag_fwd);
    m.impl("stft_mag_bwd", stft_mag_bwd);
    m.impl("mss_loss_fwd", mss_loss_fwd);
}
```

Before: 4.764 billion.

## Rewrite filtered-noise kernels as warp-per-row-pair with packed f32x2 FMA

Replaces the CTA-wide multi-row filtered-noise forward and backward kernels, and the separate noise2 path that used a global design table, with warp-specialized kernels. Each warp handles two rows packed as float pairs and uses fma2 for both rows at once, with a padded shared layout to reduce bank conflicts. The design matrix is computed per block in shared memory, and the FIR and correlation work uses 8-wide register tiling. Block-level syncs become warp syncs and the cached design-table tensor is removed. The risk is redundant per-block table setup, register pressure under a __maxnreg__(80) cap, and a large change in behaviour.

```diff
diff --git a/ddsp_pytorch_b200/csrc/noise.cu b/ddsp_pytorch_b200/csrc/noise.cu
--- a/ddsp_pytorch_b200/csrc/noise.cu
+++ b/ddsp_pytorch_b200/csrc/noise.cu
@@ -94,177 +94,324 @@
     }
 }
 
+constexpr int kNoiseWarps = 4;
+constexpr int kNoisePairsPerWarp = 4;
+
+__host__ __device__ __forceinline__ int nz_slot(int u) { return u + 2 * (u >> 4); }
+
 struct NoiseLayout {
-    int NBp, HP, F, half, bs, stride;
-    __host__ __device__ NoiseLayout(int NB, int bs_) {
-        half = NB - 1; F = 2 * half; bs = bs_;
-        NBp = (NB + 3) & ~3; HP = (half + 1 + 3) & ~3;
-        stride = NBp + HP + F + (half + bs) + bs;
-        stride = (stride + 3) & ~3;
-    }
-    __host__ __device__ int m() const { return 0; }
-    __host__ __device__ int h() const { return NBp; }
-    __host__ __device__ int taps() const { return NBp + HP; }
-    __host__ __device__ int xs() const { return NBp + HP + F; }
-    __host__ __device__ int ys() const { return NBp + HP + F + half + bs; }
+    int half, F, H8, BS8, P, C, head, xs, taps, ftaps, m, yf, gs, part, df, dh, warp;
+    __host__ __device__ NoiseLayout(int NB, int bs, bool bwd) {
+        half = NB - 1; F = 2 * half;
+        H8 = (half + 7) & ~7;
+        BS8 = (bs + 7) & ~7;
+        P = H8;
+        C = (bs + H8 - 1) / H8;
+        const int lx = P + BS8 + 8;
+        const int xsf = 2 * (nz_slot(lx) + 2);
+        head = bwd ? ((F + 3) & ~3) + ((half + 4) & ~3) : ((NB * half + 3) & ~3) + 2 * F + 2 * half;
+        xs = 0;
+        taps = ftaps = m = yf = gs = part = df = dh = 0;
+        if (!bwd) {
+            taps = xsf; ftaps = taps + 2 * (H8 + 4); m = ftaps + 2 * (H8 + 4); yf = m + 2 * ((NB + 2) & ~1);
+            warp = yf + 2 * H8;
+        } else {
+            gs = xsf; part = gs + xsf; df = part + 2 * C * H8; dh = df + 2 * H8;
+            warp = dh + 2 * half;
+        }
+    }
 };
 
-__global__ void __launch_bounds__(kNoiseThreads)
+__device__ __forceinline__ uint64_t bc2(float c) { return pk2(c, c); }
+
+__device__ __forceinline__ void ld4(uint64_t *v, const uint64_t *a, int u) {
+    const ulonglong2 *p = reinterpret_cast<const ulonglong2 *>(a + nz_slot(u));
+    const ulonglong2 x = p[0], y = p[1];
+    v[0] = x.x; v[1] = x.y; v[2] = y.x; v[3] = y.y;
+}
+__device__ __forceinline__ void ld8(uint64_t (&v)[8], const uint64_t *a, int u) {
+    ld4(v, a, u);
+    ld4(v + 4, a, u + 4);
+}
+
+__device__ __forceinline__ void stage_pairs(uint64_t *dst, const float *src, int64_t ra, bool hb, int bs, int P,
+                                            int n, int lane) {
+    for (int q = lane; q < n / 4; q += 32) {
+        const int pos = 4 * q - P;
+        float4 a = make_float4(0.f, 0.f, 0.f, 0.f), b = a;
+        if (pos >= 0 && pos < bs) {
+            a = __ldg(reinterpret_cast<const float4 *>(src + ra * bs + pos));
+            if (hb) b = __ldg(reinterpret_cast<const float4 *>(src + (ra + 1) * bs + pos));
+        }
+        float4 *d = reinterpret_cast<float4 *>(dst + nz_slot(4 * q));
+        d[0] = make_float4(a.x, b.x, a.y, b.y);
+        d[1] = make_float4(a.z, b.z, a.w, b.w);
+    }
+}
+
+__device__ __forceinline__ void cos_sum(const uint64_t *v, int len, int n, const float *ct, int F, uint64_t &ev,
+                                        uint64_t &od) {
+    ev = 0ull;
+    od = 0ull;
+    int idx = 0;
+    for (int j = 0; j < len; j += 2) {
+        const ulonglong2 m = *reinterpret_cast<const ulonglong2 *>(v + j);
+        ev = fma2(m.x, bc2(ct[idx]), ev);
+        idx += n;
+        if (idx >= F) idx -= F;
+        od = fma2(m.y, bc2(ct[idx]), od);
+        idx += n;
+        if (idx >= F) idx -= F;
+    }
+}
+
+__device__ __forceinline__ void fir_step(uint64_t (&acc)[8], const uint64_t *tp, const uint64_t (&lo)[8],
+                                         const uint64_t (&hi)[8]) {
+#pragma unroll
+    for (int t = 0; t < 8; t += 2) {
+        const ulonglong2 c = *reinterpret_cast<const ulonglong2 *>(tp + t);
+#pragma unroll
+        for (int r = 0; r < 8; ++r) {
+            acc[r] = fma2(c.x, r >= t ? hi[r - t] : lo[8 + r - t], acc[r]);
+            acc[r] = fma2(c.y, r >= t + 1 ? hi[r - t - 1] : lo[7 + r - t], acc[r]);
+        }
+    }
+}
+
+__device__ __forceinline__ void fir8(uint64_t (&acc)[8], const uint64_t *tp, const uint64_t *xs, int u0, int ntaps) {
+    uint64_t a[8], b[8];
+    ld8(a, xs, u0);
+    int d = 0;
+    for (; d + 16 <= ntaps; d += 16) {
+        ld8(b, xs, u0 - d - 8);
+        fir_step(acc, tp + d, b, a);
+        ld8(a, xs, u0 - d - 16);
+        fir_step(acc, tp + d + 8, a, b);
+    }
+    if (d < ntaps) {
+        ld8(b, xs, u0 - d - 8);
+        fir_step(acc, tp + d, b, a);
+    }
+}
+
+__device__ __forceinline__ void corr_step(uint64_t (&acc)[8], const uint64_t (&g)[8], const uint64_t (&lo)[8],
+                                          const uint64_t (&hi)[8]) {
+#pragma unroll
+    for (int u = 0; u < 8; ++u)
+#pragma unroll
+        for (int r = 0; r < 8; ++r) acc[r] = fma2(g[u], u >= r ? hi[u - r] : lo[8 + u - r], acc[r]);
+}
+
+__device__ __forceinline__ void corr8(uint64_t (&acc)[8], const uint64_t *gs, int ug, const uint64_t *xs, int ux,
+                                      int n) {
+    uint64_t a[8], b[8], g[8];
+    ld8(a, xs, ux - 8);
+    int j = 0;
+    for (; j + 16 <= n; j += 16) {
+        ld8(b, xs, ux + j);
+        ld8(g, gs, ug + j);
+        corr_step(acc, g, a, b);
+        ld8(a, xs, ux + j + 8);
+        ld8(g, gs, ug + j + 8);
+        corr_step(acc, g, b, a);
+    }
+    if (j < n) {
+        ld8(b, xs, ux + j);
+        ld8(g, gs, ug + j);
+        corr_step(acc, g, a, b);
+    }
+}
+
+__device__ __forceinline__ void noise_tables(float *smem, int half, int F) {
+    float *ct = smem, *w = smem + ((F + 3) & ~3);
+    for (int i = threadIdx.x; i < F; i += blockDim.x) ct[i] = cospif(2.f * (float)i / (float)F);
+    for (int i = threadIdx.x; i <= half; i += blockDim.x) w[i] = hann_periodic(i, F);
+    __syncthreads();
+}
+
+__device__ __forceinline__ void noise_design_columns(float *smem, int NB, int half, int F) {
+    float *D = smem;
+    double *q = reinterpret_cast<double *>(smem + ((NB * half + 3) & ~3)), *wd = q + F;
+    for (int i = threadIdx.x; i < F; i += blockDim.x) q[i] = cospi(2.0 * (double)i / F) / F;
+    for (int d = threadIdx.x; d < half; d += blockDim.x) wd[d] = 0.5 - 0.5 * cospi(2.0 * (double)(d + half) / F);
+    __syncthreads();
+    for (int d = threadIdx.x; d < half; d += blockDim.x) {
+        const double w = wd[d];
+        int idx = 0;
+        for (int k = 0; k < NB; ++k) {
+            const double ck = (k == 0 || k == half) ? 1.0 : 2.0;
+            D[k * half + d] = (float)(ck * q[idx] * w);
+            idx += d;
+            if (idx >= F) idx -= F;
+        }
+    }
+    __syncthreads();
+}
+
+__global__ void __maxnreg__(80)
 filtered_noise_fwd_kernel(const float *__restrict__ mags, const float *__restrict__ noise,
-                          const float *__restrict__ add, float *__restrict__ out, int64_t rows, int NB,
-                          int bs, int RPC, int apply_scale, float bias) {
+                          const float *__restrict__ add, float *__restrict__ out, int64_t rows, int NB, int bs,
+                          int apply_scale, float bias) {
     extern __shared__ __align__(16) float smem[];
-    const NoiseLayout L(NB, bs);
-    const int half = L.half, F = L.F;
-    float *ct = smem;
-    float *rowbase = smem + ((F + 3) & ~3);
-    const int tid = threadIdx.x;
-    for (int i = tid; i < F; i += kNoiseThreads) ct[i] = cospif(2.f * (float)i / (float)F);
-
-    const int QT = bs >> 2;
-    for (int64_t r0 = (int64_t)blockIdx.x * RPC; r0 < rows; r0 += (int64_t)gridDim.x * RPC) {
-        const int nr = (int)min((int64_t)RPC, rows - r0);
-        __syncthreads();
-        for (int i = tid; i < nr * NB; i += kNoiseThreads) {
-            const int r = i / NB, k = i - r * NB;
-            const float m = __ldg(mags + (r0 + r) * NB + k);
-            rowbase[r * L.stride + L.m() + k] = apply_scale ? ddsp_scale_fn(m + bias) : m;
-        }
-        for (int i = tid; i < nr * (half + bs); i += kNoiseThreads) {
-            const int r = i / (half + bs), j = i - r * (half + bs);
-            rowbase[r * L.stride + L.xs() + j] = j < half ? 0.f : __ldg(noise + (r0 + r) * bs + (j - half));
-        }
-        __syncthreads();
-        {
-            const int per = kNoiseThreads / nr;
-            const int r = tid / per, t = tid - r * per;
-            if (r < nr) {
-                float *rb = rowbase + r * L.stride;
-                ir_design_row(rb + L.m(), ct, rb + L.h(), NB, t, per);
+    const NoiseLayout L(NB, bs, false);
+    const int half = L.half, F = L.F, H8 = L.H8, P = L.P;
+    noise_design_columns(smem, NB, half, F);
+    const float *D = smem;
+    const int warp = threadIdx.x >> 5, lane = threadIdx.x & 31, nw = blockDim.x >> 5;
+    float *ws = smem + L.head + warp * L.warp;
+    uint64_t *xs = reinterpret_cast<uint64_t *>(ws + L.xs), *c2 = reinterpret_cast<uint64_t *>(ws + L.taps);
+    uint64_t *f2 = reinterpret_cast<uint64_t *>(ws + L.ftaps), *m2 = reinterpret_cast<uint64_t *>(ws + L.m);
+    uint64_t *yf = reinterpret_cast<uint64_t *>(ws + L.yf);
+    const int nf = H8 / 8, nitems = nf + L.BS8 / 8, s = bs - half;
+
+    for (int64_t ra = 2 * ((int64_t)blockIdx.x * nw + warp); ra < rows; ra += 2 * (int64_t)gridDim.x * nw) {
+        const bool hb = ra + 1 < rows;
+        __syncwarp();
+        stage_pairs(xs, noise, ra, hb, bs, P, P + L.BS8 + 8, lane);
+        for (int k = lane; k < NB; k += 32) {
+            float a = __ldg(mags + ra * NB + k), b = hb ? __ldg(mags + (ra + 1) * NB + k) : 0.f;
+            if (apply_scale) {
+                a = ddsp_scale_fn(a + bias);
+                b = hb ? ddsp_scale_fn(b + bias) : 0.f;
             }
-        }
-        __syncthreads();
-        for (int i = tid; i < nr * F; i += kNoiseThreads) {
-            const int r = i / F, d = i - r * F;
-            float *rb = rowbase + r * L.stride;
-            const float *h = rb + L.h();
-            rb[L.taps() + d] = d < half ? h[d] * hann_periodic(d + half, F)
-                                        : h[F - d] * hann_periodic(d - half, F);
-        }
-        __syncthreads();
-        for (int w = tid; w < nr * QT; w += kNoiseThreads) {
-            const int r = w / QT, i = (w - r * QT) * 4;
-            const float *rb = rowbase + r * L.stride;
-            const float4 *c4 = reinterpret_cast<const float4 *>(rb + L.taps());
-            const float *xs = rb + L.xs() + half + i;
-            float y0 = 0.f, y1 = 0.f, y2 = 0.f, y3 = 0.f;
-            float4 hi = *reinterpret_cast<const float4 *>(xs);
-            for (int d = 0; d < half; d += 4) {
-                const float4 lo = *reinterpret_cast<const float4 *>(xs - d - 4);
-                const float4 c = c4[d >> 2];
-                y0 = fmaf(c.x, hi.x, y0); y1 = fmaf(c.x, hi.y, y1); y2 = fmaf(c.x, hi.z, y2); y3 = fmaf(c.x, hi.w, y3);
-                y0 = fmaf(c.y, lo.w, y0); y1 = fmaf(c.y, hi.x, y1); y2 = fmaf(c.y, hi.y, y2); y3 = fmaf(c.y, hi.z, y3);
-                y0 = fmaf(c.z, lo.z, y0); y1 = fmaf(c.z, lo.w, y1); y2 = fmaf(c.z, hi.x, y2); y3 = fmaf(c.z, hi.y, y3);
-                y0 = fmaf(c.w, lo.y, y0); y1 = fmaf(c.w, lo.z, y1); y2 = fmaf(c.w, lo.w, y2); y3 = fmaf(c.w, hi.x, y3);
-                hi = lo;
+            m2[k] = pk2(a, b);
+        }
+        __syncwarp();
+        for (int d = lane; d < half; d += 32) {
+            uint64_t acc = 0ull;
+            for (int k = 0; k < NB; ++k) acc = fma2(m2[k], bc2(D[k * half + d]), acc);
+            c2[d] = acc;
+            f2[half - d] = acc;
+        }
+        if (lane == 0) f2[0] = 0ull;
+        for (int j = half + lane; j < H8; j += 32) {
+            c2[j] = 0ull;
+            if (j > half) f2[j] = 0ull;
+        }
+        __syncwarp();
+        for (int base = 0; base < nitems; base += 32) {
+            const int it = base + lane;
+            const bool far = it < nf;
+            uint64_t acc[8];
+#pragma unroll
+            for (int r = 0; r < 8; ++r) acc[r] = 0ull;
+            if (it < nitems)
+                fir8(acc, far ? f2 : c2, xs, P + 8 * (far ? it : it - nf), far ? 8 * it + 8 : H8);
+            if (far) {
+#pragma unroll
+                for (int r = 0; r < 8; ++r) yf[8 * it + r] = acc[r];
             }
-            *reinterpret_cast<float4 *>(const_cast<float *>(rb) + L.ys() + i) = make_float4(y0, y1, y2, y3);
-        }
-        __syncthreads();
-        for (int w = tid; w < nr * half; w += kNoiseThreads) {
-            const int r = w / half, t = w - r * half;
-            float *rb = rowbase + r * L.stride;
-            const float *far = rb + L.taps() + half;
-            const float *x = rb + L.xs() + half;
-            float acc = 0.f;
-            for (int e = 1; e <= t; ++e) acc = fmaf(far[e], x[t - e], acc);
-            rb[L.ys() + bs - half + t] += acc;
-        }
-        __syncthreads();
-        for (int i = tid; i < nr * bs; i += kNoiseThreads) {
-            const int r = i / bs, j = i - r * bs;
-            float y = rowbase[r * L.stride + L.ys() + j];
-            if (add) y += __ldg(add + (r0 + r) * bs + j);
-            out[(r0 + r) * bs + j] = y;
-        }
-    }
-}
-
-__global__ void __launch_bounds__(kNoiseThreads)
+            __syncwarp();
+            if (it < nitems && !far) {
+                const int i = 8 * (it - nf);
+#pragma unroll
+                for (int hq = 0; hq < 2; ++hq) {
+                    const int pos = i + 4 * hq;
+                    if (pos < bs) {
+                        float ya[4], yb[4];
+#pragma unroll
+                        for (int r = 0; r < 4; ++r) {
+                            uint64_t y = acc[4 * hq + r];
+                            if (pos >= s) y = add2(y, yf[pos - s + r]);
+                            unpk2(y, ya[r], yb[r]);
+                        }
+                        float4 oa = make_float4(ya[0], ya[1], ya[2], ya[3]);
+                        float4 ob = make_float4(yb[0], yb[1], yb[2], yb[3]);
+                        if (add) {
+                            const float4 u = __ldg(reinterpret_cast<const float4 *>(add + ra * bs + pos));
+                            oa.x += u.x; oa.y += u.y; oa.z += u.z; oa.w += u.w;
+                            if (hb) {
+                                const float4 v = __ldg(reinterpret_cast<const float4 *>(add + (ra + 1) * bs + pos));
+                                ob.x += v.x; ob.y += v.y; ob.z += v.z; ob.w += v.w;
+                            }
+                        }
+                        *reinterpret_cast<float4 *>(out + ra * bs + pos) = oa;
+                        if (hb) *reinterpret_cast<float4 *>(out + (ra + 1) * bs + pos) = ob;
+                    }
+                }
+            }
+        }
+    }
+}
+
+__global__ void __launch_bounds__(kNoiseWarps * 32)
 filtered_noise_bwd_kernel(const float *__restrict__ g_out, const float *__restrict__ noise,
-                          const float *__restrict__ mags_raw, float *__restrict__ d_mags, int64_t rows,
-                          int NB, int bs, int RPC, int apply_scale, float bias) {
+                          const float *__restrict__ mags_raw, float *__restrict__ d_mags, int64_t rows, int NB,
+                          int bs, int apply_scale, float bias) {
     extern __shared__ __align__(16) float smem[];
-    const NoiseLayout L(NB, bs);
-    const int half = L.half, F = L.F;
-    float *ct = smem;
-    float *rowbase = smem + ((F + 3) & ~3);
-    const int tid = threadIdx.x;
-    for (int i = tid; i < F; i += kNoiseThreads) ct[i] = cospif(2.f * (float)i / (float)F);
-
-    for (int64_t r0 = (int64_t)blockIdx.x * RPC; r0 < rows; r0 += (int64_t)gridDim.x * RPC) {
-        const int nr = (int)min((int64_t)RPC, rows - r0);
-        __syncthreads();
-        for (int i = tid; i < nr * (half + bs); i += kNoiseThreads) {
-            const int r = i / (half + bs), j = i - r * (half + bs);
-            rowbase[r * L.stride + L.xs() + j] = j < half ? 0.f : __ldg(noise + (r0 + r) * bs + (j - half));
-        }
-        for (int i = tid; i < nr * bs; i += kNoiseThreads) {
-            const int r = i / bs, j = i - r * bs;
-            rowbase[r * L.stride + L.ys() + j] = __ldg(g_out + (r0 + r) * bs + j);
-        }
-        __syncthreads();
-        for (int w = tid; w < nr * F; w += kNoiseThreads) {
-            const int r = w / F, d = w - r * F;
-            float *rb = rowbase + r * L.stride;
-            const float *g = rb + L.ys();
-            const float *x = rb + L.xs() + half;
-            float a0 = 0.f, a1 = 0.f;
-            if (d < half) {
-                int i = 0;
-                for (; i + 1 < bs; i += 2) {
-                    a0 = fmaf(g[i], x[i - d], a0);
-                    a1 = fmaf(g[i + 1], x[i + 1 - d], a1);
-                }
-                if (i < bs) a0 = fmaf(g[i], x[i - d], a0);
-            } else {
-                const int e = d - half;
-                if (e >= 1)
-                    for (int t = e; t < half; ++t) a0 = fmaf(g[bs - half + t], x[t - e], a0);
-            }
-            rb[L.taps() + d] = a0 + a1;
-        }
-        __syncthreads();
-        for (int w = tid; w < nr * (half + 1); w += kNoiseThreads) {
-            const int r = w / (half + 1), n = w - r * (half + 1);
-            float *rb = rowbase + r * L.stride;
-            const float *dt = rb + L.taps();
-            float v = 0.f;
-            if (n < half) v = dt[n] * hann_periodic(n + half, F);
-            const int e = half - n;
-            if (e >= 1 && e < half) v = fmaf(dt[half + e], hann_periodic(e, F), v);
-            rb[L.h() + n] = v;
-        }
-        __syncthreads();
-        {
-            const int per = kNoiseThreads / nr;
-            const int r = tid / per, t = tid - r * per;
-            if (r < nr) {
-                float *rb = rowbase + r * L.stride;
-                ir_design_row_bwd(rb + L.h(), ct, rb + L.m(), NB, t, per);
-            }
-        }
-        __syncthreads();
-        for (int i = tid; i < nr * NB; i += kNoiseThreads) {
-            const int r = i / NB, k = i - r * NB;
-            float d = rowbase[r * L.stride + L.m() + k];
-            if (apply_scale) d *= ddsp_scale_grad(__ldg(mags_raw + (r0 + r) * NB + k) + bias);
-            d_mags[(r0 + r) * NB + k] = d;
-        }
-    }
-}
-
-constexpr int kN2Threads = 256;
+    const NoiseLayout L(NB, bs, true);
+    const int half = L.half, F = L.F, H8 = L.H8, P = L.P, C = L.C;
+    noise_tables(smem, half, F);
+    const float *ct = smem, *w = smem + ((F + 3) & ~3);
+    const int warp = threadIdx.x >> 5, lane = threadIdx.x & 31;
+    const int64_t ra = 2 * ((int64_t)blockIdx.x * (blockDim.x >> 5) + warp);
+    if (ra >= rows) return;
+    const bool hb = ra + 1 < rows;
+    float *ws = smem + L.head + warp * L.warp;
+    uint64_t *xs = reinterpret_cast<uint64_t *>(ws + L.xs), *gs = reinterpret_cast<uint64_t *>(ws + L.gs);
+    uint64_t *part = reinterpret_cast<uint64_t *>(ws + L.part), *df = reinterpret_cast<uint64_t *>(ws + L.df);
+    uint64_t *dh = reinterpret_cast<uint64_t *>(ws + L.dh);
+
+    stage_pairs(xs, noise, ra, hb, bs, P, P + L.BS8 + 8, lane);
+    stage_pairs(gs, g_out, ra, hb, bs, P, P + L.BS8 + 8, lane);
+    __syncwarp();
+    const int nb = H8 / 8, ng = L.BS8 / 8, nmain = nb * C, nitems = nmain + nb, s = bs - half;
+    for (int base = 0; base < nitems; base += 32) {
+        const int it = base + lane;
+        if (it < nitems) {
+            const bool far = it >= nmain;
+            const int c = far ? 0 : it / nb, b = far ? it - nmain : it - c * nb;
+            const int g0 = c * ng / C, g1 = (c + 1) * ng / C;
+            uint64_t acc[8];
+#pragma unroll
+            for (int r = 0; r < 8; ++r) acc[r] = 0ull;
+            corr8(acc, gs, far ? P + s + 8 * b : P + 8 * g0, xs, far ? P : P + 8 * (g0 - b),
+                  far ? H8 - 8 * b : 8 * (g1 - g0));
+            uint64_t *dst = far ? df + 8 * b : part + c * H8 + 8 * b;
+#pragma unroll
+            for (int r = 0; r < 8; ++r) dst[r] = acc[r];
+        }
+    }
+    __syncwarp();
+    float mida = 0.f, midb = 0.f;
+    for (int n = lane; n < half; n += 32) {
+        uint64_t v = part[n];
+        for (int c = 1; c < C; ++c) v = add2(v, part[c * H8 + n]);
+        if (n >= 1) v = add2(v, df[half - n]);
+        v = fma2(v, bc2(w[half - n]), 0ull);
+        dh[n] = v;
+        if (!(n & 1)) {
+            float a, b;
+            unpk2(v, a, b);
+            const float sg = (n & 2) ? -1.f : 1.f;
+            mida = fmaf(sg, a, mida);
+            midb = fmaf(sg, b, midb);
+        }
+    }
+    mida = ddsp_warp_sum(mida);
+    midb = ddsp_warp_sum(midb);
+    __syncwarp();
+    const float invF = 1.f / (float)F;
+    auto store = [&](int k, float a, float b) {
+        if (apply_scale) a *= ddsp_scale_grad(__ldg(mags_raw + ra * NB + k) + bias);
+        d_mags[ra * NB + k] = a;
+        if (hb) {
+            if (apply_scale) b *= ddsp_scale_grad(__ldg(mags_raw + (ra + 1) * NB + k) + bias);
+            d_mags[(ra + 1) * NB + k] = b;
+        }
+    };
+    for (int k = lane; k < half / 2; k += 32) {
+        uint64_t ev, od;
+        cos_sum(dh, half, k, ct, F, ev, od);
+        float a0, b0, a1, b1;
+        unpk2(add2(ev, od), a0, b0);
+        unpk2(fma2(bc2(-1.f), od, ev), a1, b1);
+        const float ck = (k == 0 ? 1.f : 2.f) * invF;
+        store(k, a0 * ck, b0 * ck);
+        store(half - k, a1 * ck, b1 * ck);
+    }
+    if (lane == 0) store(half / 2, mida * 2.f * invF, midb * 2.f * invF);
+}
 
 __global__ void noise_design_kernel(float *__restrict__ tab, int NB) {
     const int half = NB - 1, F = 2 * half, NBq = (NB + 3) & ~3;
@@ -286,243 +433,6 @@
     }
 }
 
-__device__ __forceinline__ float4 fir4(const float4 *__restrict__ t4, const float *x, int ntaps) {
-    float y0 = 0.f, y1 = 0.f, y2 = 0.f, y3 = 0.f;
-    float4 hi = *reinterpret_cast<const float4 *>(x);
-    for (int d = 0; d < ntaps; d += 4) {
-        const float4 lo = *reinterpret_cast<const float4 *>(x - d - 4);
-        const float4 c = t4[d >> 2];
-        y0 = fmaf(c.x, hi.x, y0); y1 = fmaf(c.x, hi.y, y1); y2 = fmaf(c.x, hi.z, y2); y3 = fmaf(c.x, hi.w, y3);
-        y0 = fmaf(c.y, lo.w, y0); y1 = fmaf(c.y, hi.x, y1); y2 = fmaf(c.y, hi.y, y2); y3 = fmaf(c.y, hi.z, y3);
-        y0 = fmaf(c.z, lo.z, y0); y1 = fmaf(c.z, lo.w, y1); y2 = fmaf(c.z, hi.x, y2); y3 = fmaf(c.z, hi.y, y3);
-        y0 = fmaf(c.w, lo.y, y0); y1 = fmaf(c.w, lo.z, y1); y2 = fmaf(c.w, lo.w, y2); y3 = fmaf(c.w, hi.x, y3);
-        hi = lo;
-    }
-    return make_float4(y0, y1, y2, y3);
-}
-
-__device__ __forceinline__ float4 corr4(const float *g, const float *x, int d, int len) {
-    float a0 = 0.f, a1 = 0.f, a2 = 0.f, a3 = 0.f;
-    float4 lo = *reinterpret_cast<const float4 *>(x - d - 4);
-    for (int i = 0; i < len; i += 4) {
-        const float4 hi = *reinterpret_cast<const float4 *>(x + i - d);
-        const float4 gv = *reinterpret_cast<const float4 *>(g + i);
-        a0 = fmaf(gv.x, hi.x, a0); a0 = fmaf(gv.y, hi.y, a0); a0 = fmaf(gv.z, hi.z, a0); a0 = fmaf(gv.w, hi.w, a0);
-        a1 = fmaf(gv.x, lo.w, a1); a1 = fmaf(gv.y, hi.x, a1); a1 = fmaf(gv.z, hi.y, a1); a1 = fmaf(gv.w, hi.z, a1);
-        a2 = fmaf(gv.x, lo.z, a2); a2 = fmaf(gv.y, lo.w, a2); a2 = fmaf(gv.z, hi.x, a2); a2 = fmaf(gv.w, hi.y, a2);
-        a3 = fmaf(gv.x, lo.y, a3); a3 = fmaf(gv.y, lo.z, a3); a3 = fmaf(gv.z, lo.w, a3); a3 = fmaf(gv.w, hi.x, a3);
-        lo = hi;
-    }
-    return make_float4(a0, a1, a2, a3);
-}
-
-struct Noise2Layout {
-    int half, F, NBq, bs, xs_len, stride;
-    __host__ __device__ Noise2Layout(int NB, int bs_) {
-        half = NB - 1; F = 2 * half; NBq = (NB + 3) & ~3; bs = bs_;
-        xs_len = half + bs;
-        stride = NBq + F + xs_len + bs + half;
-    }
-    __host__ __device__ int m() const { return 0; }
-    __host__ __device__ int taps() const { return NBq; }
-    __host__ __device__ int xs() const { return NBq + F; }
-    __host__ __device__ int ys() const { return NBq + F + xs_len; }
-    __host__ __device__ int yf() const { return NBq + F + xs_len + bs; }
-};
-
-__global__ void __launch_bounds__(kN2Threads)
-filtered_noise2_fwd_kernel(const float *__restrict__ mags, const float *__restrict__ noise,
-                           const float *__restrict__ add, const float *__restrict__ design,
-                           float *__restrict__ out, int64_t rows, int NB, int bs, int RPC, int apply_scale,
-                           float bias) {
-    extern __shared__ __align__(16) float smem[];
-    const Noise2Layout L(NB, bs);
-    const int half = L.half, F = L.F;
-    float *D = smem;
-    float *rowbase = D + NB * F;
-    const int tid = threadIdx.x, warp = tid >> 5, lane = tid & 31;
-    constexpr int NW = kN2Threads / 32;
-    for (int i = tid; i < NB * F / 4; i += kN2Threads)
-        reinterpret_cast<float4 *>(D)[i] = __ldg(reinterpret_cast<const float4 *>(design) + i);
-
-    const int QM = bs >> 2, QF = half >> 2;
-    for (int64_t r0 = (int64_t)blockIdx.x * RPC; r0 < rows; r0 += (int64_t)gridDim.x * RPC) {
-        const int nr = (int)min((int64_t)RPC, rows - r0);
-        __syncthreads();
-        for (int r = warp; r < nr; r += NW) {
-            float *rb = rowbase + r * L.stride;
-            const float *mg = mags + (r0 + r) * NB;
-            for (int k = lane; k < NB; k += 32) {
-                const float m = __ldg(mg + k);
-                rb[L.m() + k] = apply_scale ? ddsp_scale_fn(m + bias) : m;
-            }
-            for (int j = lane; j < half; j += 32) rb[L.xs() + j] = 0.f;
-            const float4 *nz = reinterpret_cast<const float4 *>(noise + (r0 + r) * bs);
-            float4 *xs4 = reinterpret_cast<float4 *>(rb + L.xs() + half);
-            for (int j = lane; j < QM; j += 32) xs4[j] = __ldg(nz + j);
-        }
-        __syncthreads();
-        for (int it = tid; it < ((nr + 1) >> 1) * (F / 4); it += kN2Threads) {
-            const int rp = it / (F / 4), c = it - rp * (F / 4);
-            const int ra = 2 * rp, rb_ = min(2 * rp + 1, nr - 1);
-            const float *ma = rowbase + ra * L.stride + L.m();
-            const float *mb = rowbase + rb_ * L.stride + L.m();
-            const float4 *d4 = reinterpret_cast<const float4 *>(D) + c;
-            float4 a = make_float4(0.f, 0.f, 0.f, 0.f), e = a;
-#define DDSP_N2_MAC(X, Y, U)                                                                                  \
-    a.x = fmaf(X, U.x, a.x); a.y = fmaf(X, U.y, a.y); a.z = fmaf(X, U.z, a.z); a.w = fmaf(X, U.w, a.w);      \
-    e.x = fmaf(Y, U.x, e.x); e.y = fmaf(Y, U.y, e.y); e.z = fmaf(Y, U.z, e.z); e.w = fmaf(Y, U.w, e.w);
-            for (int k = 0; k < NB - 1; k += 4) {
-                const float4 xa = *reinterpret_cast<const float4 *>(ma + k);
-                const float4 xb = *reinterpret_cast<const float4 *>(mb + k);
-                const float4 u0 = d4[k * (F / 4)], u1 = d4[(k + 1) * (F / 4)];
-                const float4 u2 = d4[(k + 2) * (F / 4)], u3 = d4[(k + 3) * (F / 4)];
-                DDSP_N2_MAC(xa.x, xb.x, u0)
-                DDSP_N2_MAC(xa.y, xb.y, u1)
-                DDSP_N2_MAC(xa.z, xb.z, u2)
-                DDSP_N2_MAC(xa.w, xb.w, u3)
-            }
-            {
-                const float4 u = d4[(NB - 1) * (F / 4)];
-                const float x = ma[NB - 1], y = mb[NB - 1];
-                DDSP_N2_MAC(x, y, u)
-            }
-#undef DDSP_N2_MAC
-            reinterpret_cast<float4 *>(rowbase + ra * L.stride + L.taps())[c] = a;
-            if (rb_ != ra) reinterpret_cast<float4 *>(rowbase + rb_ * L.stride + L.taps())[c] = e;
-        }
-        __syncthreads();
-        const int nmain = nr * QM;
-        for (int it = tid; it < nmain + nr * QF; it += kN2Threads) {
-            if (it < nmain) {
-                const int r = it / QM, q = it - r * QM;
-                float *rb = rowbase + r * L.stride;
-                const float4 y = fir4(reinterpret_cast<const float4 *>(rb + L.taps()), rb + L.xs() + half + 4 * q, half);
-                *reinterpret_cast<float4 *>(rb + L.ys() + 4 * q) = y;
-            } else {
-                const int i2 = it - nmain;
-                const int r = i2 / QF, qq = i2 - r * QF;
-                float *rb = rowbase + r * L.stride;
-                const float4 y = fir4(reinterpret_cast<const float4 *>(rb + L.taps()) + QF,
-                                      rb + L.xs() + half + 4 * qq, half);
-                *reinterpret_cast<float4 *>(rb + L.yf() + 4 * qq) = y;
-            }
-        }
-        __syncthreads();
-        for (int r = warp; r < nr; r += NW) {
-            const float *rb = rowbase + r * L.stride;
-            const float4 *ys4 = reinterpret_cast<const float4 *>(rb + L.ys());
-            const float4 *yf4 = reinterpret_cast<const float4 *>(rb + L.yf());
-            const float4 *ad4 = add ? reinterpret_cast<const float4 *>(add + (r0 + r) * bs) : nullptr;
-            float4 *o4 = reinterpret_cast<float4 *>(out + (r0 + r) * bs);
-            for (int j = lane; j < QM; j += 32) {
-                float4 y = ys4[j];
-                if (j >= QM - QF) {
-                    const float4 f = yf4[j - (QM - QF)];
-                    y.x += f.x; y.y += f.y; y.z += f.z; y.w += f.w;
-                }
-                if (ad4) {
-                    const float4 f = __ldg(ad4 + j);
-                    y.x += f.x; y.y += f.y; y.z += f.z; y.w += f.w;
-                }
-                o4[j] = y;
-            }
-        }
-    }
-}
-
-__global__ void __launch_bounds__(kN2Threads)
-filtered_noise2_bwd_kernel(const float *__restrict__ g_out, const float *__restrict__ noise,
-                           const float *__restrict__ mags_raw, const float *__restrict__ design,
-                           float *__restrict__ d_mags, int64_t rows, int NB, int bs, int RPC,
-                           int apply_scale, float bias) {
-    extern __shared__ __align__(16) float smem[];
-    const Noise2Layout L(NB, bs);
-    const int half = L.half, F = L.F, NBq = L.NBq;
-    float *Dt = smem;
-    float *rowbase = Dt + F * NBq;
-    const int tid = threadIdx.x, warp = tid >> 5, lane = tid & 31;
-    constexpr int NW = kN2Threads / 32;
-    const float *dt_src = design + (size_t)NB * F;
-    for (int i = tid; i < F * NBq / 4; i += kN2Threads)
-        reinterpret_cast<float4 *>(Dt)[i] = __ldg(reinterpret_cast<const float4 *>(dt_src) + i);
-    const int QM = bs >> 2;
-
-    for (int64_t r0 = (int64_t)blockIdx.x * RPC; r0 < rows; r0 += (int64_t)gridDim.x * RPC) {
-        const int nr = (int)min((int64_t)RPC, rows - r0);
-        __syncthreads();
-        for (int r = warp; r < nr; r += NW) {
-            float *rb = rowbase + r * L.stride;
-            for (int j = lane; j < half; j += 32) rb[L.xs() + j] = 0.f;
-            const float4 *nz = reinterpret_cast<const float4 *>(noise + (r0 + r) * bs);
-            const float4 *gz = reinterpret_cast<const float4 *>(g_out + (r0 + r) * bs);
-            float4 *xs4 = reinterpret_cast<float4 *>(rb + L.xs() + half);
-            float4 *g4 = reinterpret_cast<float4 *>(rb + L.ys());
-            for (int j = lane; j < QM; j += 32) {
-                xs4[j] = __ldg(nz + j);
-                g4[j] = __ldg(gz + j);
-            }
-        }
-        __syncthreads();
-        const int ncausal = nr * (half / 4);
-        for (int it = tid; it < 2 * ncausal; it += kN2Threads) {
-            const bool far = it >= ncausal;
-            const int i2 = far ? it - ncausal : it;
-            const int r = i2 / (half / 4), tg = i2 - r * (half / 4);
-            float *rb = rowbase + r * L.stride;
-            const float *x = rb + L.xs() + half;
-            const float4 a = far ? corr4(rb + L.ys() + bs - half, x, 4 * tg, half) : corr4(rb + L.ys(), x, 4 * tg, bs);
-            *reinterpret_cast<float4 *>(rb + L.taps() + (far ? half : 0) + 4 * tg) = a;
-        }
-        __syncthreads();
-        for (int it = tid; it < ((nr + 1) >> 1) * (NBq / 4); it += kN2Threads) {
-            const int rp = it / (NBq / 4), kg = it - rp * (NBq / 4);
-            const int ra = 2 * rp, rb_ = min(2 * rp + 1, nr - 1);
-            const float *ta = rowbase + ra * L.stride + L.taps();
-            const float *tb = rowbase + rb_ * L.stride + L.taps();
-            const float4 *d4 = reinterpret_cast<const float4 *>(Dt) + kg;
-            float4 a = make_float4(0.f, 0.f, 0.f, 0.f), e = a;
-#define DDSP_N2_MAC(X, Y, U)                                                                                  \
-    a.x = fmaf(X, U.x, a.x); a.y = fmaf(X, U.y, a.y); a.z = fmaf(X, U.z, a.z); a.w = fmaf(X, U.w, a.w);      \
-    e.x = fmaf(Y, U.x, e.x); e.y = fmaf(Y, U.y, e.y); e.z = fmaf(Y, U.z, e.z); e.w = fmaf(Y, U.w, e.w);
-            for (int j = 0; j < F; j += 4) {
-                const float4 xa = *reinterpret_cast<const float4 *>(ta + j);
-                const float4 xb = *reinterpret_cast<const float4 *>(tb + j);
-                const float4 u0 = d4[j * (NBq / 4)], u1 = d4[(j + 1) * (NBq / 4)];
-                const float4 u2 = d4[(j + 2) * (NBq / 4)], u3 = d4[(j + 3) * (NBq / 4)];
-                DDSP_N2_MAC(xa.x, xb.x, u0)
-                DDSP_N2_MAC(xa.y, xb.y, u1)
-                DDSP_N2_MAC(xa.z, xb.z, u2)
-                DDSP_N2_MAC(xa.w, xb.w, u3)
-            }
-#undef DDSP_N2_MAC
-#pragma unroll
-            for (int h2 = 0; h2 < 2; ++h2) {
-                if (h2 == 1 && rb_ == ra) break;
-                const int r = h2 ? rb_ : ra;
-                const float4 acc = h2 ? e : a;
-                const float av[4] = {acc.x, acc.y, acc.z, acc.w};
-#pragma unroll
-                for (int q = 0; q < 4; ++q) {
-                    const int k = 4 * kg + q;
-                    if (k < NB) {
-                        float d = av[q];
-                        if (apply_scale) d *= ddsp_scale_grad(__ldg(mags_raw + (r0 + r) * NB + k) + bias);
-                        d_mags[(r0 + r) * NB + k] = d;
-                    }
-                }
-            }
-        }
-    }
-}
-
-inline int noise_rows_per_cta(int bs) {
-    int rpc = (kNoiseThreads * 4) / bs;
-    if (rpc < 1) rpc = 1;
-    if (rpc > 8) rpc = 8;
-    return rpc;
-}
-
 }
 
 extern "C" int ddsp_b200_amp_to_ir_fwd(const float *amp, float *ir, int64_t rows, int NB, int target,
@@ -549,30 +459,17 @@
     return ddsp_launch_status();
 }
 
-static int noise_launch_cfg(int64_t rows, int NB, int bs, int *rpc, size_t *smem, int *grid) {
-    if (NB < 3 || (NB - 1) % 4 != 0) return DDSP_B200_EUNSUPPORTED;
+static int noise_plan(int64_t rows, int NB, int bs, bool bwd, int *warps, size_t *smem, int64_t *grid) {
+    if (NB < 5 || (NB - 1) % 4 != 0) return DDSP_B200_EUNSUPPORTED;
     if (bs % 4 != 0 || bs < 2 * (NB - 1)) return DDSP_B200_EUNSUPPORTED;
-    *rpc = noise_rows_per_cta(bs);
-    const NoiseLayout L(NB, bs);
-    *smem = ((size_t)((L.F + 3) & ~3) + (size_t)*rpc * L.stride) * sizeof(float);
+    const NoiseLayout L(NB, bs, bwd);
+    int w = kNoiseWarps;
+    while (w > 1 && ((size_t)L.head + (size_t)w * L.warp) * sizeof(float) > 200 * 1024) w >>= 1;
+    *smem = ((size_t)L.head + (size_t)w * L.warp) * sizeof(float);
     if (*smem > 200 * 1024) return DDSP_B200_EUNSUPPORTED;
-    const int64_t ctas = ddsp_ceil_div(rows, *rpc);
-    *grid = (int)(ctas < DDSP_SM_COUNT * 8 ? ctas : DDSP_SM_COUNT * 8);
+    *warps = w;
+    *grid = ddsp_ceil_div(ddsp_ceil_div(rows, 2), (int64_t)w * (bwd ? 1 : kNoisePairsPerWarp));
     return DDSP_B200_OK;
-}
-
-static bool noise2_cfg(int64_t rows, int NB, int bs, bool bwd, int *rpc, size_t *smem, int *grid) {
-    if (NB < 5 || (NB - 1) % 4 != 0 || bs % 4 != 0 || bs < 2 * (NB - 1)) return false;
-    const Noise2Layout L(NB, bs);
-    const size_t fixed = (bwd ? (size_t)L.F * L.NBq : (size_t)NB * L.F) * sizeof(float);
-    int r = 16;
-    while (r > 1 && fixed + (size_t)r * L.stride * sizeof(float) > 75 * 1024) r >>= 1;
-    *smem = fixed + (size_t)r * L.stride * sizeof(float);
-    if (*smem > 200 * 1024) return false;
-    *rpc = r;
-    const int64_t ctas = ddsp_ceil_div(rows, r);
-    *grid = (int)(ctas < DDSP_SM_COUNT * 3 ? ctas : DDSP_SM_COUNT * 3);
-    return true;
 }
 
 extern "C" int64_t ddsp_b200_noise_design_size(int NB) {
@@ -590,25 +487,18 @@
 extern "C" int ddsp_b200_filtered_noise_fwd(const float *mags, const float *noise, const float *add,
                                             const float *design, float *out, int64_t rows, int NB,
                                             int block_size, int apply_scale, float bias, void *stream) {
+    (void)design;
     DDSP_REQUIRE(mags && noise && out && rows >= 0);
     if (rows == 0) return DDSP_B200_OK;
-    int rpc, grid;
+    int warps;
     size_t smem;
-    if (design && noise2_cfg(rows, NB, block_size, false, &rpc, &smem, &grid)) {
-        if (smem > 48 * 1024)
-            cudaFuncSetAttribute(filtered_noise2_fwd_kernel, cudaFuncAttributeMaxDynamicSharedMemorySize,
-                                 (int)smem);
-        filtered_noise2_fwd_kernel<<<grid, kN2Threads, smem, (cudaStream_t)stream>>>(
-            mags, noise, add, design, out, rows, NB, block_size, rpc, apply_scale, bias);
-        return ddsp_launch_status();
-    }
-    int s = noise_launch_cfg(rows, NB, block_size, &rpc, &smem, &grid);
+    int64_t grid;
+    const int s = noise_plan(rows, NB, block_size, false, &warps, &smem, &grid);
     if (s) return s;
     if (smem > 48 * 1024)
-        cudaFuncSetAttribute(filtered_noise_fwd_kernel, cudaFuncAttributeMaxDynamicSharedMemorySize,
-                             (int)smem);
-    filtered_noise_fwd_kernel<<<grid, kNoiseThreads, smem, (cudaStream_t)stream>>>(
-        mags, noise, add, out, rows, NB, block_size, rpc, apply_scale, bias);
+        cudaFuncSetAttribute(filtered_noise_fwd_kernel, cudaFuncAttributeMaxDynamicSharedMemorySize, (int)smem);
+    filtered_noise_fwd_kernel<<<(unsigned)grid, warps * 32, smem, (cudaStream_t)stream>>>(
+        mags, noise, add, out, rows, NB, block_size, apply_scale, bias);
     return ddsp_launch_status();
 }
 
@@ -616,24 +506,17 @@
                                             const float *mags_raw, const float *design, float *d_mags,
                                             int64_t rows, int NB, int block_size, int apply_scale,
                                             float bias, void *stream) {
+    (void)design;
     DDSP_REQUIRE(g_out && noise && d_mags && rows >= 0 && (!apply_scale || mags_raw));
     if (rows == 0) return DDSP_B200_OK;
-    int rpc, grid;
+    int warps;
     size_t smem;
-    if (design && noise2_cfg(rows, NB, block_size, true, &rpc, &smem, &grid)) {
-        if (smem > 48 * 1024)
-            cudaFuncSetAttribute(filtered_noise2_bwd_kernel, cudaFuncAttributeMaxDynamicSharedMemorySize,
-                                 (int)smem);
-        filtered_noise2_bwd_kernel<<<grid, kN2Threads, smem, (cudaStream_t)stream>>>(
-            g_out, noise, mags_raw, design, d_mags, rows, NB, block_size, rpc, apply_scale, bias);
-        return ddsp_launch_status();
-    }
-    int s = noise_launch_cfg(rows, NB, block_size, &rpc, &smem, &grid);
+    int64_t grid;
+    const int s = noise_plan(rows, NB, block_size, true, &warps, &smem, &grid);
     if (s) return s;
     if (smem > 48 * 1024)
-        cudaFuncSetAttribute(filtered_noise_bwd_kernel, cudaFuncAttributeMaxDynamicSharedMemorySize,
-                             (int)smem);
-    filtered_noise_bwd_kernel<<<grid, kNoiseThreads, smem, (cudaStream_t)stream>>>(
-        g_out, noise, mags_raw, d_mags, rows, NB, block_size, rpc, apply_scale, bias);
+        cudaFuncSetAttribute(filtered_noise_bwd_kernel, cudaFuncAttributeMaxDynamicSharedMemorySize, (int)smem);
+    filtered_noise_bwd_kernel<<<(unsigned)grid, warps * 32, smem, (cudaStream_t)stream>>>(
+        g_out, noise, mags_raw, d_mags, rows, NB, block_size, apply_scale, bias);
     return ddsp_launch_status();
 }
diff --git a/ddsp_pytorch_b200/csrc/torch_ops.cpp b/ddsp_pytorch_b200/csrc/torch_ops.cpp
--- a/ddsp_pytorch_b200/csrc/torch_ops.cpp
+++ b/ddsp_pytorch_b200/csrc/torch_ops.cpp
@@ -69,20 +69,6 @@
         check(ddsp_b200_fft_stage_twiddles(fpm(t), (int)n_fft, cur_stream()), "stft_stage_twiddles");
         finish_table_build("fft_stage_twiddles");
     }
-    cache[key] = t;
-    return t;
-}
-
-Tensor noise_design_table(const at::Device &dev, int64_t NB) {
-    static std::mutex mu;
-    static std::map<std::pair<int, int64_t>, Tensor> cache;
-    std::lock_guard<std::mutex> lock(mu);
-    auto key = std::make_pair((int)dev.index(), NB);
-    auto it = cache.find(key);
-    if (it != cache.end()) return it->second;
-    Tensor t = at::empty({ddsp_b200_noise_design_size((int)NB)}, at::TensorOptions().device(dev).dtype(at::kFloat));
-    check(ddsp_b200_noise_design_table(fpm(t), (int)NB, cur_stream()), "noise_design_table");
-    finish_table_build("noise_design_table");
     cache[key] = t;
     return t;
 }
@@ -401,8 +387,7 @@
     c10::cuda::CUDAGuard guard(mags.device());
     Tensor out = at::empty({B, T * bs, 1}, mags.options());
     if (B * T == 0) return out;
-    Tensor design = noise_design_table(mags.device(), NB);
-    check(ddsp_b200_filtered_noise_fwd(fp(mags), fp(noise), opt_fp(add), fp(design), fpm(out), B * T, (int)NB,
+    check(ddsp_b200_filtered_noise_fwd(fp(mags), fp(noise), opt_fp(add), nullptr, fpm(out), B * T, (int)NB,
                                        (int)bs, apply_scale, (float)bias, cur_stream()),
           "filtered_noise_fwd");
     return out;
@@ -418,8 +403,7 @@
     c10::cuda::CUDAGuard guard(noise.device());
     Tensor d_mags = at::empty({B, T, NB}, noise.options());
     if (B * T == 0) return d_mags;
-    Tensor design = noise_design_table(noise.device(), NB);
-    check(ddsp_b200_filtered_noise_bwd(fp(g), fp(noise), opt_fp(raw), fp(design), fpm(d_mags), B * T, (int)NB,
+    check(ddsp_b200_filtered_noise_bwd(fp(g), fp(noise), opt_fp(raw), nullptr, fpm(d_mags), B * T, (int)NB,
                                        (int)bs, apply_scale, (float)bias, cur_stream()),
           "filtered_noise_bwd");
     return d_mags;
```

Result: faster. 4.870 billion, median of 6 (+2.2%).
